# zailaiyiwan123/NOVA_pointcloud

Measured on AMD Instinct MI355X. Metric: generated points/sec/node, NOVA-d48w1024 @2048 pts, 64-step sample, higher is better.
Workload: dtype bf16; 1 GPU; d48w1024_2048pts_b32; ar_steps=64, diffusion_steps=25, batch_per_gpu=32, global_batch=32, guidance=cfg 2-pass, process_group=none

## Files before the change

include/nova_hip.h:

```cpp
#ifndef NOVA_HIP_H_
#define NOVA_HIP_H_

#ifdef __cplusplus
extern "C" {
#endif

#define NOVA_HIP_VERSION 404

typedef enum { NOVA_F32 = 0, NOVA_BF16 = 1, NOVA_F16 = 2 } nova_dtype;
typedef enum { NOVA_ACT_NONE = 0, NOVA_ACT_GELU_ERF = 1, NOVA_ACT_SILU = 2 } nova_act;
typedef enum {
  NOVA_OK = 0,
  NOVA_ERR_ARG = -1,
  NOVA_ERR_SHAPE = -2,
  NOVA_ERR_LAUNCH = -3,
  NOVA_ERR_DEVICE = -4
} nova_status;

int nova_version(void);
const char* nova_last_error(void);
int nova_check_device(void);

#define NOVA_PROF_SLOTS 10
int nova_prof_enable(int on);
int nova_prof_collect(double* ms, double* work, long long* launches, int slots);

int nova_debug_force_gemm_tile(int tile);

int nova_debug_set_attn_variant(int variant);

int nova_debug_set_graphs(int on);
int nova_debug_graph_stats(long* captures, long* replays);
int nova_debug_drop_graphs(void);

int nova_gemm_bias_act(const void* A, const void* W, const float* bias, void* out, int M, int N, int K, int act,
                       int dtype, void* stream);

int nova_quantize_rows_fp8(const void* x_bf16, void* out_fp8, float* scale, long long rows, int D, void* stream);
int nova_gemm_fp8_bias_act(const void* A8, const float* a_scale, const void* W8, const float* w_scale, const float* bias,
                           void* out_bf16, int M, int N, int K, int act, void* stream);

int nova_qkv_rope(const void* x, const void* Wqkv, const float* bias, const float* rope, void* qkv, int S, int L, int D,
                  int heads, int rope_batch, int dtype, void* stream);

int nova_qkv_rope_cols(const void* x, const void* W, const float* bias, const float* rope, void* out, int M, int N, int K,
                       int L, int rope_batch, int head_dim, int rope_cols, int dtype, void* stream);

int nova_rope_table(const float* pos, const long long* ids, float* rope, int nb, int pad, int n_tok, int n_pos, int hd,
                    const float* inv_freq, void* stream);

int nova_attn_fwd(const void* q, const void* k, const void* v, void* o, int S, int heads, int Lq, int Lk, int head_dim,
                  long q_row_stride, long kv_row_stride, long o_row_stride, float scale, int dtype, void* stream);

int nova_attn_fwd_lse(const void* q_scaled, const void* k, const void* v, void* o, float* lse, int S, int heads, int L,
                      int head_dim, long qkv_row_stride, long o_row_stride, const int* key_limit, void* stream);
int nova_attn_bwd(const void* q_scaled, const void* k, const void* v, const void* o, const void* d_o, const float* lse,
                  float* delta_scratch, void* dq, void* dk, void* dv, int S, int heads, int L, int head_dim,
                  long qkv_row_stride, long o_row_stride, long do_row_stride, long dqkv_row_stride, float scale,
                  const int* key_limit, void* stream);

int nova_act_fwd(const void* x, void* y, long long n, int kind, int dtype, void* stream);
int nova_act_bwd(const void* x, const void* dy, void* dx, long long n, int kind, int dtype, void* stream);

int nova_row_norm_bwd(const void* x, const void* dy, const float* gamma, const float* beta, const void* mod, long mod_ld,
                      int scale_off, int shift_off, int gate_off, void* dx, void* dmod, float* dgamma_part, float* dbeta_part,
                      int parts, long rows, int D, float eps, int dtype, void* stream);

int nova_row_norm(const void* in, void* out, const float* gamma, const float* beta, const void* mod, long mod_ld,
                  int scale_off, int shift_off, int gate_off, const void* res, const int* gather, long rows, int D,
                  float eps, int dtype, void* stream);

int nova_row_norm_chain(const void* g, const void* x, const float* gamma, const float* beta, const void* mod, long mod_ld,
                        int gate_off, int scale_off, int shift_off, float eps_first, float eps_second, void* x_new_out,
                        void* h_out, long rows, int D, int dtype, void* stream);

int nova_adaln_fc1(const void* x, const void* mod, long mod_ld, int scale_off, int shift_off, float eps, const void* w,
                   const float* bias, void* h, void* out, long rows, int N, int D, int act, int dtype, void* stream);

int nova_embed_canvas(const float* canvas, const float* mask, const void* w, const float* bias, const void* mask_token,
                      const void* pos_embed, void* z0, int B, int N, int P, int D, int dtype, void* stream);
int nova_build_sequence(const void* prefix, long prefix_seq_rows, const void* tokens, long tok_batch_rows,
                        const long long* ids, void* x, int S, int B, int Lp, int n_sel, int D, int dtype, void* stream);
int nova_scatter_tokens(const void* x1, const long long* ids, void* x2, int S, int B, int Lp, int N, int n_prev, int D,
                        int dtype, void* stream);

int nova_silu_add_rows(const void* a, const void* rowvec, void* out, long rows, int D, int dtype, void* stream);
int nova_timestep_freq(const float* t, const float* freq, void* out, int n, int freq_dim, int dtype, void* stream);
int nova_patch_embed_rows(const float* x, const void* w, const float* bias, void* out, int S, int B, int n, int P, int D,
                          int dtype, void* stream);
int nova_head_cfg_euler(const void* h, const void* w, const float* bias, float* x, int B, int n, int P, int D,
                        float guidance, int cfg, float dt, int dtype, void* stream);

int nova_pointset_nn_dist(const float* x, const float* y, float* d, int B, int N, int M, float clamp_lo, float clamp_hi,
                          int unit_norm, void* stream);
int nova_pointset_pairwise_dist(const float* x, const float* y, float* D, int B, int N, int M, float clamp_lo, float clamp_hi,
                                void* stream);
int nova_pointset_chamfer_matrix(const float* x, const float* y, float* cd, int A, int B, int N, int M, int ldc, int symmetric,
                                 void* stream);
#define NOVA_EMD_MAX_POINTS 4096
int nova_pointset_emd_matrix(const float* x, const float* y, float* emd, int A, int B, int N, int ldc, void* stream);

#define NOVA_OCC_MAX_RES 32
int nova_pointset_occupancy_grid(const float* x, long long* counters, long long* bernoulli, int* node, long long* outside, int S,
                                 int N, int R, int in_sphere, int workgroups, void* stream);

typedef struct {
  const void* qkv_w;
  const float* qkv_b;
  const void* proj_w;
  const float* proj_b;
  const float* norm1_w;
  const float* norm1_b;
  const void* fc1_w;
  const float* fc1_b;
  const void* fc2_w;
  const float* fc2_b;
  const float* norm2_w;
  const float* norm2_b;
} nova_vit_block;

int nova_vit_blocks_forward(const nova_vit_block* blocks, int nblocks, void* x, int S, int L, int D, int heads,
                            int hidden, const float* rope, int rope_batch, void* ws_qkv, void* ws_a, void* ws_b,
                            void* ws_h, int dtype, void* stream);

typedef struct {
  const void* qkv_w8;  const float* qkv_ws;
  const void* fc1_w8;  const float* fc1_ws;
  const void* fc2_w8;  const float* fc2_ws;
} nova_vit_block_fp8;

int nova_row_norm_fp8(const void* in, void* out, const float* gamma, const float* beta, const void* res, void* out8, float* out8_scale,
                      long rows, int D, float eps, void* stream);
int nova_gemm_fp8_gelu_q8(const void* A8, const float* a_scale, const void* W8, const float* w_scale, const float* bias, void* out8,
                          int M, int N, int K, const float* out_scale, unsigned* out_amax, void* stream);
int nova_qkv_rope_fp8(const void* x8, const float* x_scale, const void* w8, const float* w_scale, const float* bias, const float* rope,
                      void* qkv, int S, int L, int D, int heads, int rope_batch, float q_scale, void* stream);

int nova_vit_blocks_forward_fp8(const nova_vit_block* blocks, const nova_vit_block_fp8* q, int nblocks, void* x, int S, int L, int D,
                                int heads, int hidden, const float* rope, int rope_batch, void* ws_qkv, void* ws_a, void* ws_b,
                                void* ws_h, void* ws_x8, float* ws_xs, void* ws_h8, float* ws_hs, float* h_scale, unsigned* h_amax,
                                void* stream);

int nova_vit_blocks_forward_kv(const nova_vit_block* blocks, int nblocks, void* x, int S, int L, int D, int heads,
                               int hidden, const float* rope, int rope_batch, void* kv_cache, long cache_cap,
                               long cache_len, void* ws_qkv, void* ws_a, void* ws_b, void* ws_h, int dtype, void* stream);

int nova_modulate_rows(const void* x, const void* mod, void* out, long rows, int D, int dtype, void* stream);

typedef struct {
  const void* fc1_w;
  const float* fc1_b;
  const void* fc2_w;
  const float* fc2_b;
  const float* norm2_w;
  const float* norm2_b;
} nova_mlp_block;

typedef struct {
  int depth;
  const nova_mlp_block* blocks;
  const void* adaln_w;
  const float* adaln_b;
  const void* patch_w;
  const float* patch_b;
  const void* head_w;
  const float* head_b;
} nova_decoder;

typedef struct {
  float guidance, kx, kv, clip, c0, cx, sigma;
  float extra_scale;
  int extra_kind;
} nova_sampler_step;

int nova_decoder_denoise(const nova_decoder* dec, const void* zc, const void* temb, float* x, const nova_sampler_step* sched,
                         const float* noise, float renorm, float* echo_energy, int steps, int S, int B, int n, int P, int D,
                         void* ws_a, void* ws_u, void* ws_h, void* ws_f, void* ws_g, void* ws_mod, float* ws_v, int mod_steps,
                         int dtype, void* stream);

int nova_decoder_denoise_echo(const nova_decoder* dec, const void* zc, const void* temb, float* x, const nova_sampler_step* sched,
                              const float* noise, float renorm, float* echo_rows, const float* echo_noise, int Ne, int steps, int S, int B,
                              int n, int P, int D, void* ws_a, void* ws_u, void* ws_h, void* ws_f, void* ws_g, void* ws_mod, float* ws_v,
                              int mod_steps, int dtype, void* stream);

#ifdef __cplusplus
}
#endif
#endif
```

nova_pointcloud_amd/csrc/capi.hip:

```cpp
#include <cstdarg>
#include <cstdio>
#include <cstring>
#include <atomic>
#include <cmath>
#include <cstdlib>
#include <mutex>
#include <string>
#include <unordered_map>
#include <utility>
#include <vector>
#include "common.h"
#include "nova_internal.h"

namespace nova {

static thread_local char g_err[512] = "";

int set_error(int code, const char* fmt, ...) {
  va_list ap;
  va_start(ap, fmt);
  vsnprintf(g_err, sizeof(g_err), fmt, ap);
  va_end(ap);
  return code;
}

int check_launch(const char* what) {
  const hipError_t e = hipGetLastError();
  if (e == hipSuccess) return 0;
  return set_error(NOVA_ERR_LAUNCH, "%s: %s", what, hipGetErrorString(e));
}

struct ProfRec { hipEvent_t a, b; int slot; double work; };
static std::atomic<bool> g_prof_on{false};
static std::mutex g_prof_mu;
static std::vector<ProfRec> g_prof;
static std::vector<std::pair<hipEvent_t, hipEvent_t>> g_prof_pool;

ProfScope::ProfScope(int slot, double work, hipStream_t s) : idx(-1), st(s) {
  if (!g_prof_on.load(std::memory_order_relaxed)) return;
  std::lock_guard<std::mutex> lk(g_prof_mu);
  ProfRec r;
  if (!g_prof_pool.empty()) {
    r.a = g_prof_pool.back().first;
    r.b = g_prof_pool.back().second;
    g_prof_pool.pop_back();
  } else if (hipEventCreate(&r.a) != hipSuccess || hipEventCreate(&r.b) != hipSuccess) {
    return;
  }
  r.slot = slot;
  r.work = work;
  (void)hipEventRecord(r.a, st);
  g_prof.push_back(r);
  idx = (int)g_prof.size() - 1;
}
ProfScope::~ProfScope() {
  if (idx < 0) return;
  std::lock_guard<std::mutex> lk(g_prof_mu);
  if (idx < (int)g_prof.size()) (void)hipEventRecord(g_prof[idx].b, st);
}

static inline bool bad_dtype(int dtype) { return dtype != NOVA_F32 && dtype != NOVA_BF16 && dtype != NOVA_F16; }
static inline size_t esize(int dtype) { return dtype_is16(dtype) ? 2 : 4; }

}

using namespace nova;

#define NOVA_REQUIRE(cond, code, ...) \
  do {                                \
    if (!(cond)) return set_error(code, __VA_ARGS__); \
  } while (0)
#define NOVA_TRY(expr)        \
  do {                        \
    const int rc_ = (expr);   \
    if (rc_ != 0) return rc_; \
  } while (0)

namespace nova {
static thread_local bool g_walk_rev = false;
void walk_reverse(bool on) { g_walk_rev = on; }
bool walk_is_reverse() { return g_walk_rev; }
#ifdef NOVA_EXPERIMENTS
static int g_walk_alternate = 1;
void walk_set_alternate(int on) { g_walk_alternate = on; }
#else
constexpr int g_walk_alternate = 1;
#endif
}

extern "C" {

int nova_version(void) { return NOVA_HIP_VERSION; }
const char* nova_last_error(void) { return g_err; }

int nova_check_device(void) {
  int dev = -1;
  if (hipGetDevice(&dev) != hipSuccess) return set_error(NOVA_ERR_DEVICE, "no HIP device");
  hipDeviceProp_t prop;
  if (hipGetDeviceProperties(&prop, dev) != hipSuccess) return set_error(NOVA_ERR_DEVICE, "hipGetDeviceProperties failed");
  if (strncmp(prop.gcnArchName, "gfx950", 6) != 0)
    return set_error(NOVA_ERR_DEVICE, "device %d is %s; libnova_hip is built for gfx950 only", dev, prop.gcnArchName);
  return 0;
}

int nova_debug_force_gemm_tile(int tile) {
  NOVA_REQUIRE(gemm_force_tile(tile) == 0, NOVA_ERR_ARG,
               "force_gemm_tile: this build knows 0 (auto), 16 (small-M kernel; 161 / 162 / 164 with 16 / 32 / 64 rows per workgroup), 64 / 128 (the small-M tile kernels), 256 (persistent), 257 (one tile per workgroup) and 258 (persistent, prologue form); experiment codes need the NOVA_EXPERIMENTS build");
  return 0;
}

int nova_prof_enable(int on) {
  g_prof_on.store(on != 0);
  return 0;
}

int nova_prof_collect(double* ms, double* work, long long* launches, int slots) {
  NOVA_REQUIRE(ms && work && launches && slots >= PROF_SLOTS, NOVA_ERR_ARG, "prof_collect: need %d slots", PROF_SLOTS);
  for (int i = 0; i < slots; ++i) { ms[i] = 0; work[i] = 0; launches[i] = 0; }
  std::lock_guard<std::mutex> lk(g_prof_mu);
  for (auto& r : g_prof) {
    float t = 0.f;
    if (hipEventSynchronize(r.b) == hipSuccess && hipEventElapsedTime(&t, r.a, r.b) == hipSuccess) {
      ms[r.slot] += t;
      work[r.slot] += r.work;
      launches[r.slot] += 1;
    }
    g_prof_pool.emplace_back(r.a, r.b);
  }
  g_prof.clear();
  return 0;
}

int nova_gemm_bias_act(const void* A, const void* W, const float* bias, void* out, int M, int N, int K, int act,
                       int dtype, void* stream) {
  NOVA_REQUIRE(!bad_dtype(dtype), NOVA_ERR_ARG, "gemm: bad dtype %d", dtype);
  NOVA_REQUIRE(M == 0 || (A && W && out), NOVA_ERR_ARG, "gemm: null pointer");
  return gemm_bias_act(A, W, bias, out, M, N, K, act, dtype, (hipStream_t)stream);
}

int nova_quantize_rows_fp8(const void* x, void* out, float* scale, long long rows, int D, void* stream) {
  NOVA_REQUIRE(rows <= 0 || (x && out && scale), NOVA_ERR_ARG, "quantize_rows_fp8: null pointer");
  return quantize_rows_fp8(x, out, scale, (long)rows, D, (hipStream_t)stream);
}

int nova_gemm_fp8_bias_act(const void* A8, const float* a_scale, const void* W8, const float* w_scale, const float* bias,
                           void* out, int M, int N, int K, int act, void* stream) {
  NOVA_REQUIRE(M <= 0 || (A8 && a_scale && W8 && w_scale && out), NOVA_ERR_ARG, "gemm_fp8: null pointer");
  NOVA_REQUIRE(act >= NOVA_ACT_NONE && act <= NOVA_ACT_SILU, NOVA_ERR_ARG, "gemm_fp8: bad activation %d", act);
  return gemm256_fp8_launch(A8, a_scale, W8, w_scale, bias, out, M, N, K, act, (hipStream_t)stream);
}

int nova_qkv_rope(const void* x, const void* Wqkv, const float* bias, const float* rope, void* qkv, int S, int L, int D,
                  int heads, int rope_batch, int dtype, void* stream) {
  NOVA_REQUIRE(!bad_dtype(dtype), NOVA_ERR_ARG, "qkv_rope: bad dtype %d", dtype);
  NOVA_REQUIRE(S * L == 0 || (x && Wqkv && qkv), NOVA_ERR_ARG, "qkv_rope: null pointer");
  return gemm_qkv_rope(x, Wqkv, bias, rope, qkv, S, L, D, heads, rope_batch, dtype, (hipStream_t)stream);
}

int nova_qkv_rope_cols(const void* x, const void* W, const float* bias, const float* rope, void* out, int M, int N, int K,
                       int L, int rope_batch, int head_dim, int rope_cols, int dtype, void* stream) {
  NOVA_REQUIRE(!bad_dtype(dtype), NOVA_ERR_ARG, "qkv_rope_cols: bad dtype %d", dtype);
  NOVA_REQUIRE(M == 0 || (x && W && out), NOVA_ERR_ARG, "qkv_rope_cols: null pointer");
  NOVA_REQUIRE(L > 0 && head_dim > 0 && head_dim % 4 == 0 && rope_cols % 128 == 0 && rope_cols <= N, NOVA_ERR_SHAPE,
               "qkv_rope_cols: bad L/head_dim/rope_cols");
  return gemm_rope_cols(x, W, bias, rope, out, M, N, K, L, rope_batch, head_dim, rope_cols, dtype, (hipStream_t)stream);
}

int nova_rope_table(const float* pos, const long long* ids, float* rope, int nb, int pad, int n_tok, int n_pos, int hd,
                    const float* inv_freq, void* stream) {
  NOVA_REQUIRE(pos && rope && inv_freq, NOVA_ERR_ARG, "rope_table: null pointer");
  NOVA_REQUIRE(hd > 0 && hd % 8 == 0, NOVA_ERR_SHAPE, "rope_table: head_dim %d", hd);
  return rope_table(pos, ids, rope, nb, pad, n_tok, n_pos, hd, inv_freq, (hipStream_t)stream);
}

int nova_attn_fwd(const void* q, const void* k, const void* v, void* o, int S, int heads, int Lq, int Lk, int head_dim,
                  long q_row_stride, long kv_row_stride, long o_row_stride, float scale, int dtype, void* stream) {
  NOVA_REQUIRE(!bad_dtype(dtype), NOVA_ERR_ARG, "attn_fwd: bad dtype %d", dtype);
  NOVA_REQUIRE(q && k && v && o, NOVA_ERR_ARG, "attn_fwd: null pointer");
  return attn_fwd(q, k, v, o, S, heads, Lq, Lk, head_dim, q_row_stride, kv_row_stride, o_row_stride, scale, dtype,
                  (hipStream_t)stream);
}

int nova_attn_fwd_lse(const void* q_scaled, const void* k, const void* v, void* o, float* lse, int S, int heads, int L,
                      int head_dim, long qkv_row_stride, long o_row_stride, const int* key_limit, void* stream) {
  NOVA_REQUIRE(q_scaled && k && v && o && lse, NOVA_ERR_ARG, "attn_fwd_lse: null pointer");
  return attn_fwd(q_scaled, k, v, o, S, heads, L, L, head_dim, qkv_row_stride, qkv_row_stride, o_row_stride, 1.0f, NOVA_BF16,
                  (hipStream_t)stream, true, 0, lse, key_limit);
}

int nova_attn_bwd(const void* q_scaled, const void* k, const void* v, const void* o, const void* d_o, const float* lse,
                  float* delta_scratch, void* dq, void* dk, void* dv, int S, int heads, int L, int head_dim,
                  long qkv_row_stride, long o_row_stride, long do_row_stride, long dqkv_row_stride, float scale,
                  const int* key_limit, void* stream) {
  NOVA_REQUIRE(q_scaled && k && v && o && d_o && lse && delta_scratch && dq && dk && dv, NOVA_ERR_ARG, "attn_bwd: null pointer");
  return attn_bwd(q_scaled, k, v, o, d_o, lse, delta_scratch, dq, dk, dv, S, heads, L, head_dim, qkv_row_stride, o_row_stride,
                  do_row_stride, dqkv_row_stride, scale, (hipStream_t)stream, key_limit);
}

int nova_row_norm(const void* in, void* out, const float* gamma, const float* beta, const void* mod, long mod_ld,
                  int scale_off, int shift_off, int gate_off, const void* res, const int* gather, long rows, int D,
                  float eps, int dtype, void* stream) {
  NOVA_REQUIRE(!bad_dtype(dtype), NOVA_ERR_ARG, "row_norm: bad dtype %d", dtype);
  NOVA_REQUIRE(rows == 0 || (in && out), NOVA_ERR_ARG, "row_norm: null pointer");
  RowNormArgs a{in, out, gamma, beta, mod, mod_ld, scale_off, shift_off, gate_off, res, gather, rows, D, eps};
  return row_norm(a, dtype, (hipStream_t)stream);
}

int nova_row_norm_chain(const void* g, const void* x, const float* gamma, const float* beta, const void* mod, long mod_ld,
                        int gate_off, int scale_off, int shift_off, float eps_first, float eps_second, void* x_new_out,
                        void* h_out, long rows, int D, int dtype, void* stream) {
  NOVA_REQUIRE(dtype_is16(dtype), NOVA_ERR_ARG, "row_norm_chain: dtype %d is not a 16-bit storage type", dtype);
  NOVA_REQUIRE(rows == 0 || (g && x && mod && h_out), NOVA_ERR_ARG, "row_norm_chain: null pointer");
  RowNormArgs a2{g, nullptr, gamma, beta, mod, mod_ld, -1, -1, gate_off, x, nullptr, rows, D, eps_first};
  RowNormArgs a1{nullptr, h_out, nullptr, nullptr, mod, mod_ld, scale_off, shift_off, -1, nullptr, nullptr, rows, D, eps_second};
  return row_norm_chain(a2, a1, x_new_out, dtype, (hipStream_t)stream);
}

int nova_adaln_fc1(const void* x, const void* mod, long mod_ld, int scale_off, int shift_off, float eps, const void* w,
                   const float* bias, void* h, void* out, long rows, int N, int D, int act, int dtype, void* stream) {
  NOVA_REQUIRE(!bad_dtype(dtype), NOVA_ERR_ARG, "adaln_fc1: bad dtype %d", dtype);
  NOVA_REQUIRE(rows == 0 || (x && mod && w && h && out), NOVA_ERR_ARG, "adaln_fc1: null pointer");
  NOVA_REQUIRE(rows >= 0 && rows <= 0x7fffffffL && scale_off >= 0 && shift_off >= 0, NOVA_ERR_ARG, "adaln_fc1: bad rows / offsets");
  RowNormArgs m{x, h, nullptr, nullptr, mod, mod_ld, scale_off, shift_off, -1, nullptr, nullptr, rows, D, eps};
  return gemm_modulate_act(m, w, bias, out, (int)rows, N, D, act, dtype, (hipStream_t)stream);
}

int nova_embed_canvas(const float* canvas, const float* mask, const void* w, const float* bias, const void* mask_token,
                      const void* pos_embed, void* z0, int B, int N, int P, int D, int dtype, void* stream) {
  NOVA_REQUIRE(!bad_dtype(dtype), NOVA_ERR_ARG, "embed_canvas: bad dtype %d", dtype);
  NOVA_REQUIRE(canvas && mask && w && bias && mask_token && z0, NOVA_ERR_ARG, "embed_canvas: null pointer");
  return embed_canvas(canvas, mask, w, bias, mask_token, pos_embed, z0, B, N, P, D, dtype, (hipStream_t)stream);
}

int nova_build_sequence(const void* prefix, long prefix_seq_rows, const void* tokens, long tok_batch_rows,
                        const long long* ids, void* x, int S, int B, int Lp, int n_sel, int D, int dtype, void* stream) {
  NOVA_REQUIRE(!bad_dtype(dtype), NOVA_ERR_ARG, "build_sequence: bad dtype %d", dtype);
  NOVA_REQUIRE(x && (Lp == 0 || prefix) && (n_sel == 0 || tokens) && B > 0, NOVA_ERR_ARG, "build_sequence: null pointer");
  return build_sequence(prefix, prefix_seq_rows, tokens, tok_batch_rows, ids, x, S, B, Lp, n_sel, D, dtype, (hipStream_t)stream);
}

int nova_scatter_tokens(const void* x1, const long long* ids, void* x2, int S, int B, int Lp, int N, int n_prev, int D,
                        int dtype, void* stream) {
  NOVA_REQUIRE(!bad_dtype(dtype), NOVA_ERR_ARG, "scatter_tokens: bad dtype %d", dtype);
  NOVA_REQUIRE(n_prev == 0 || (x1 && ids && x2 && B > 0), NOVA_ERR_ARG, "scatter_tokens: null pointer");
  return scatter_tokens(x1, ids, x2, S, B, Lp, N, n_prev, D, dtype, (hipStream_t)stream);
}

int nova_silu_add_rows(const void* a, const void* rowvec, void* out, long rows, int D, int dtype, void* stream) {
  NOVA_REQUIRE(!bad_dtype(dtype), NOVA_ERR_ARG, "silu_add_rows: bad dtype %d", dtype);
  NOVA_REQUIRE(rows == 0 || (a && out), NOVA_ERR_ARG, "silu_add_rows: null pointer");
  return silu_add_rows(a, rowvec, out, rows, D, dtype, (hipStream_t)stream);
}

int nova_timestep_freq(const float* t, const float* freq, void* out, int n, int freq_dim, int dtype, void* stream) {
  NOVA_REQUIRE(!bad_dtype(dtype), NOVA_ERR_ARG, "timestep_freq: bad dtype %d", dtype);
  NOVA_REQUIRE(t && freq && out && freq_dim % 2 == 0, NOVA_ERR_ARG, "timestep_freq: bad argument");
  return timestep_freq(t, freq, out, n, freq_dim, dtype, (hipStream_t)stream);
}

int nova_patch_embed_rows(const float* x, const void* w, const float* bias, void* out, int S, int B, int n, int P, int D,
                          int dtype, void* stream) {
  NOVA_REQUIRE(!bad_dtype(dtype), NOVA_ERR_ARG, "patch_embed_rows: bad dtype %d", dtype);
  NOVA_REQUIRE(x && w && bias && out && B > 0, NOVA_ERR_ARG, "patch_embed_rows: null pointer");
  return patch_embed_rows(x, w, bias, out, S, B, n, P, D, dtype, (hipStream_t)stream);
}

int nova_head_cfg_euler(const void* h, const void* w, const float* bias, float* x, int B, int n, int P, int D,
                        float guidance, int cfg, float dt, int dtype, void* stream) {
  NOVA_REQUIRE(!bad_dtype(dtype), NOVA_ERR_ARG, "head_cfg_euler: bad dtype %d", dtype);
  NOVA_REQUIRE(h && w && bias && x, NOVA_ERR_ARG, "head_cfg_euler: null pointer");
  NOVA_REQUIRE(!cfg || guidance > 1.0f, NOVA_ERR_ARG, "head_cfg_euler: cfg needs guidance > 1");
  SamplerStep sp{cfg ? guidance : 1.0f, 0.f, 1.f, 0.f, dt, 1.f, 0.f, 0.f, 0};
  return head_cfg_step(h, w, bias, x, nullptr, nullptr, nullptr, nullptr, B, n, P, D, sp, 0, dtype, (hipStream_t)stream);
}


static int vit_blocks(const nova_vit_block* blocks, int nblocks, void* x, int S, int L, int D, int heads, int hidden,
                      const float* rope, int rope_batch, void* ws_qkv, void* ws_a, void* ws_b, void* ws_h, void* cache,
                      long cap, long cache_len, int dtype, hipStream_t st) {
  const int M = S * L, hd = D / heads;
  if (M == 0) return 0;
  const size_t es = esize(dtype);
  const float scale = 1.0f / sqrtf((float)hd);
  const char* qkv = static_cast<const char*>(ws_qkv);
  struct Walk {
    int k = 0;
    void next() { walk_reverse(g_walk_alternate && (k++ & 1)); }
    ~Walk() { walk_reverse(false); }
  } walk;
  for (int i = 0; i < nblocks; ++i) {
    const nova_vit_block& b = blocks[i];
    const bool pre = dtype_is16(dtype);
    walk.next();
    NOVA_TRY(gemm_qkv_rope(x, b.qkv_w, b.qkv_b, rope, ws_qkv, S, L, D, heads, rope_batch, dtype, st,
                           pre ? scale * 1.4426950408889634f : 1.0f));
    walk.next();
    if (cache) {
      char* cb = static_cast<char*>(cache) + (size_t)i * S * cap * 2 * D * es;
      NOVA_TRY(kv_append(ws_qkv, cb, S, L, D, cap, cache_len, dtype, st));
      NOVA_TRY(attn_fwd(qkv, cb, cb + (size_t)D * es, ws_a, S, heads, L, (int)(cache_len + L), hd, 3L * D, 2L * D, D, scale, dtype,
                        st, pre, cap * 2L * D));
    } else {
      NOVA_TRY(attn_fwd(qkv, qkv + (size_t)D * es, qkv + (size_t)2 * D * es, ws_a, S, heads, L, L, hd, 3L * D, 3L * D, D,
                        scale, dtype, st, pre));
    }
    walk.next();
    NOVA_TRY(gemm_bias_act(ws_a, b.proj_w, b.proj_b, ws_b, M, D, D, NOVA_ACT_NONE, dtype, st));
    RowNormArgs n1{ws_b, x, b.norm1_w, b.norm1_b, nullptr, 0, -1, -1, -1, x, nullptr, M, D, 1e-5f};
    walk.next();
    NOVA_TRY(row_norm(n1, dtype, st));
    walk.next();
    NOVA_TRY(gemm_bias_act(x, b.fc1_w, b.fc1_b, ws_h, M, hidden, D, NOVA_ACT_GELU_ERF, dtype, st));
    walk.next();
    NOVA_TRY(gemm_bias_act(ws_h, b.fc2_w, b.fc2_b, ws_b, M, D, hidden, NOVA_ACT_NONE, dtype, st));
    RowNormArgs n2{ws_b, x, b.norm2_w, b.norm2_b, nullptr, 0, -1, -1, -1, x, nullptr, M, D, 1e-5f};
    walk.next();
    NOVA_TRY(row_norm(n2, dtype, st));
  }
  return 0;
}

int nova_vit_blocks_forward(const nova_vit_block* blocks, int nblocks, void* x, int S, int L, int D, int heads,
                            int hidden, const float* rope, int rope_batch, void* ws_qkv, void* ws_a, void* ws_b,
                            void* ws_h, int dtype, void* stream) {
  NOVA_REQUIRE(!bad_dtype(dtype), NOVA_ERR_ARG, "vit_blocks: bad dtype %d", dtype);
  NOVA_REQUIRE(nblocks == 0 || (blocks && x && ws_qkv && ws_a && ws_b && ws_h), NOVA_ERR_ARG, "vit_blocks: null pointer");
  NOVA_REQUIRE(heads > 0 && D % heads == 0, NOVA_ERR_SHAPE, "vit_blocks: D %% heads != 0");
  return vit_blocks(blocks, nblocks, x, S, L, D, heads, hidden, rope, rope_batch, ws_qkv, ws_a, ws_b, ws_h, nullptr, 0, 0, dtype,
                    (hipStream_t)stream);
}

int nova_row_norm_fp8(const void* in, void* out, const float* gamma, const float* beta, const void* res, void* out8, float* out8_scale,
                      long rows, int D, float eps, void* stream) {
  NOVA_REQUIRE(rows == 0 || (in && out && out8 && out8_scale), NOVA_ERR_ARG, "row_norm_fp8: null pointer");
  RowNormArgs a{in, out, gamma, beta, nullptr, 0, -1, -1, -1, res, nullptr, rows, D, eps};
  a.out8 = out8;
  a.out8_scale = out8_scale;
  return row_norm(a, NOVA_BF16, (hipStream_t)stream);
}

int nova_gemm_fp8_gelu_q8(const void* A8, const float* a_scale, const void* W8, const float* w_scale, const float* bias, void* out8,
                          int M, int N, int K, const float* out_scale, unsigned* out_amax, void* stream) {
  NOVA_REQUIRE(M <= 0 || (A8 && a_scale && W8 && w_scale && out8 && out_scale && out_amax), NOVA_ERR_ARG, "gemm_fp8_gelu_q8: null pointer");
  return gemm256_fp8_launch(A8, a_scale, W8, w_scale, bias, out8, M, N, K, NOVA_EPI_GELU_Q8, (hipStream_t)stream, nullptr, 1, 1, 2, 0, 1.0f,
                            0, 0, out_scale, out_amax);
}

int nova_qkv_rope_fp8(const void* x8, const float* x_scale, const void* w8, const float* w_scale, const float* bias, const float* rope,
                      void* qkv, int S, int L, int D, int heads, int rope_batch, float q_scale, void* stream) {
  NOVA_REQUIRE(S * L == 0 || (x8 && x_scale && w8 && w_scale && qkv), NOVA_ERR_ARG, "qkv_rope_fp8: null pointer");
  NOVA_REQUIRE(heads > 0 && D % heads == 0, NOVA_ERR_SHAPE, "qkv_rope_fp8: D %% heads != 0");
  return gemm256_fp8_launch(x8, x_scale, w8, w_scale, bias, qkv, S * L, 3 * D, D, 3, (hipStream_t)stream, rope, L, rope_batch, D / heads,
                            rope ? 2 * D : 0, q_scale, q_scale != 1.0f ? D : 0);
}

int nova_vit_blocks_forward_fp8(const nova_vit_block* blocks, const nova_vit_block_fp8* q, int nblocks, void* x, int S, int L, int D,
                                int heads, int hidden, const float* rope, int rope_batch, void* ws_qkv, void* ws_a, void* ws_b,
                                void* ws_h, void* ws_x8, float* ws_xs, void* ws_h8, float* ws_hs, float* h_scale, unsigned* h_amax,
                                void* stream) {
  NOVA_REQUIRE(nblocks == 0 || (blocks && q && x && ws_qkv && ws_a && ws_b && ws_h && ws_x8 && ws_xs && ws_h8 && ws_hs), NOVA_ERR_ARG,
               "vit_blocks_fp8: null pointer");
  NOVA_REQUIRE((h_scale == nullptr) == (h_amax == nullptr), NOVA_ERR_ARG, "vit_blocks_fp8: h_scale and h_amax come together");
  NOVA_REQUIRE(heads > 0 && D % heads == 0, NOVA_ERR_SHAPE, "vit_blocks_fp8: D %% heads != 0");
  NOVA_REQUIRE(D % 256 == 0 && hidden % 256 == 0, NOVA_ERR_SHAPE, "vit_blocks_fp8: D and hidden must be multiples of 256");
  NOVA_REQUIRE(!rope || L >= 16, NOVA_ERR_SHAPE, "vit_blocks_fp8: L >= 16 with RoPE");
  hipStream_t st = (hipStream_t)stream;
  const int M = S * L, hd = D / heads;
  if (M == 0 || nblocks == 0) return 0;
  const float scale = 1.0f / sqrtf((float)hd);
  const char* qkv = static_cast<const char*>(ws_qkv);
  struct Walk {
    int k = 0;
    void next() { walk_reverse(g_walk_alternate && (k++ & 1)); }
    ~Walk() { walk_reverse(false); }
  } walk;
  NOVA_TRY(quantize_rows_fp8(x, ws_x8, ws_xs, M, D, st));
  for (int i = 0; i < nblocks; ++i) {
    const nova_vit_block& b = blocks[i];
    const nova_vit_block_fp8& w = q[i];
    walk.next();
    NOVA_TRY(gemm256_fp8_launch(ws_x8, ws_xs, w.qkv_w8, w.qkv_ws, b.qkv_b, ws_qkv, M, 3 * D, D, 3 , st, rope, L,
                                rope_batch, hd, rope ? 2 * D : 0, scale * 1.4426950408889634f, D));
    walk.next();
    NOVA_TRY(attn_fwd(qkv, qkv + (size_t)D * 2, qkv + (size_t)2 * D * 2, ws_a, S, heads, L, L, hd, 3L * D, 3L * D, D, scale, NOVA_BF16,
                      st, true));
    walk.next();
    NOVA_TRY(gemm_bias_act(ws_a, b.proj_w, b.proj_b, ws_b, M, D, D, NOVA_ACT_NONE, NOVA_BF16, st));
    RowNormArgs n1{ws_b, x, b.norm1_w, b.norm1_b, nullptr, 0, -1, -1, -1, x, nullptr, M, D, 1e-5f};
    n1.out8 = ws_x8;
    n1.out8_scale = ws_xs;
    walk.next();
    NOVA_TRY(row_norm(n1, NOVA_BF16, st));
    walk.next();
    if (h_scale) {
      NOVA_TRY(gemm256_fp8_launch(ws_x8, ws_xs, w.fc1_w8, w.fc1_ws, b.fc1_b, ws_h8, M, hidden, D, NOVA_EPI_GELU_Q8, st, nullptr, 1, 1, 2, 0,
                                  1.0f, 0, 0, h_scale + i, h_amax + i));
      walk.next();
      NOVA_TRY(gemm256_fp8_launch(ws_h8, h_scale + i, w.fc2_w8, w.fc2_ws, b.fc2_b, ws_b, M, D, hidden, NOVA_ACT_NONE, st, nullptr, 1, 1, 2, 0,
                                  1.0f, 0, 1));
    } else {
      NOVA_TRY(gemm256_fp8_launch(ws_x8, ws_xs, w.fc1_w8, w.fc1_ws, b.fc1_b, ws_h, M, hidden, D, NOVA_ACT_GELU_ERF, st));
      NOVA_TRY(quantize_rows_fp8(ws_h, ws_h8, ws_hs, M, hidden, st));
      walk.next();
      NOVA_TRY(gemm256_fp8_launch(ws_h8, ws_hs, w.fc2_w8, w.fc2_ws, b.fc2_b, ws_b, M, D, hidden, NOVA_ACT_NONE, st));
    }
    RowNormArgs n2{ws_b, x, b.norm2_w, b.norm2_b, nullptr, 0, -1, -1, -1, x, nullptr, M, D, 1e-5f};
    if (i + 1 < nblocks) {
      n2.out8 = ws_x8;
      n2.out8_scale = ws_xs;
    }
    walk.next();
    NOVA_TRY(row_norm(n2, NOVA_BF16, st));
  }
  return 0;
}

int nova_vit_blocks_forward_kv(const nova_vit_block* blocks, int nblocks, void* x, int S, int L, int D, int heads,
                               int hidden, const float* rope, int rope_batch, void* kv_cache, long cache_cap,
                               long cache_len, void* ws_qkv, void* ws_a, void* ws_b, void* ws_h, int dtype, void* stream) {
  NOVA_REQUIRE(!bad_dtype(dtype), NOVA_ERR_ARG, "vit_blocks_kv: bad dtype %d", dtype);
  NOVA_REQUIRE(nblocks == 0 || (blocks && x && kv_cache && ws_qkv && ws_a && ws_b && ws_h), NOVA_ERR_ARG, "vit_blocks_kv: null pointer");
  NOVA_REQUIRE(heads > 0 && D % heads == 0, NOVA_ERR_SHAPE, "vit_blocks_kv: D %% heads != 0");
  NOVA_REQUIRE(cache_len >= 0 && cache_len + L <= cache_cap, NOVA_ERR_SHAPE, "vit_blocks_kv: %ld cached + %d new rows exceed the capacity %ld",
               cache_len, L, cache_cap);
  return vit_blocks(blocks, nblocks, x, S, L, D, heads, hidden, rope, rope_batch, ws_qkv, ws_a, ws_b, ws_h, kv_cache, cache_cap,
                    cache_len, dtype, (hipStream_t)stream);
}

int nova_pointset_nn_dist(const float* x, const float* y, float* d, int B, int N, int M, float clamp_lo, float clamp_hi,
                          int unit_norm, void* stream) {
  NOVA_REQUIRE(B * (long)N == 0 || (x && y && d), NOVA_ERR_ARG, "pointset_nn_dist: null pointer");
  NOVA_REQUIRE(clamp_lo <= clamp_hi, NOVA_ERR_ARG, "pointset_nn_dist: empty clamp range");
  return pointset_nn_dist(x, y, d, B, N, M, clamp_lo, clamp_hi, unit_norm, (hipStream_t)stream);
}

int nova_pointset_pairwise_dist(const float* x, const float* y, float* D, int B, int N, int M, float clamp_lo, float clamp_hi,
                                void* stream) {
  NOVA_REQUIRE(B * (long)N * M == 0 || (x && y && D), NOVA_ERR_ARG, "pointset_pairwise_dist: null pointer");
  NOVA_REQUIRE(clamp_lo <= clamp_hi, NOVA_ERR_ARG, "pointset_pairwise_dist: empty clamp range");
  return pointset_pairwise_dist(x, y, D, B, N, M, clamp_lo, clamp_hi, (hipStream_t)stream);
}

int nova_pointset_chamfer_matrix(const float* x, const float* y, float* cd, int A, int B, int N, int M, int ldc, int symmetric,
                                 void* stream) {
  NOVA_REQUIRE(A <= 0 || B <= 0 || (x && y && cd), NOVA_ERR_ARG, "pointset_chamfer_matrix: null pointer");
  NOVA_REQUIRE(ldc >= B, NOVA_ERR_ARG, "pointset_chamfer_matrix: ldc %d < B %d", ldc, B);
  NOVA_REQUIRE(!symmetric || (x == y && A == B && N == M), NOVA_ERR_ARG,
               "pointset_chamfer_matrix: symmetric mode needs x == y, A == B and N == M");
  return pointset_chamfer_matrix(x, y, cd, A, B, N, M, ldc, symmetric, (hipStream_t)stream);
}

int nova_pointset_emd_matrix(const float* x, const float* y, float* emd, int A, int B, int N, int ldc, void* stream) {
  NOVA_REQUIRE(A <= 0 || B <= 0 || (x && y && emd), NOVA_ERR_ARG, "pointset_emd_matrix: null pointer");
  NOVA_REQUIRE(ldc >= B, NOVA_ERR_ARG, "pointset_emd_matrix: ldc %d < B %d", ldc, B);
  NOVA_REQUIRE(N >= 1 && N <= NOVA_EMD_MAX_POINTS, NOVA_ERR_ARG,
               "pointset_emd_matrix: N %d outside 1 .. %d (the maximum point count NOVA_EMD_MAX_POINTS)", N, NOVA_EMD_MAX_POINTS);
  return pointset_emd_matrix(x, y, emd, A, B, N, ldc, (hipStream_t)stream);
}

int nova_pointset_occupancy_grid(const float* x, long long* counters, long long* bernoulli, int* node, long long* outside, int S,
                                 int N, int R, int in_sphere, int workgroups, void* stream) {
  return pointset_occupancy_grid(x, counters, bernoulli, node, outside, S, N, R, in_sphere, workgroups, (hipStream_t)stream);
}

int nova_modulate_rows(const void* x, const void* mod, void* out, long rows, int D, int dtype, void* stream) {
  NOVA_REQUIRE(!bad_dtype(dtype), NOVA_ERR_ARG, "modulate_rows: bad dtype %d", dtype);
  NOVA_REQUIRE(rows == 0 || (x && mod && out), NOVA_ERR_ARG, "modulate_rows: null pointer");
  return modulate_rows(x, mod, out, rows, D, dtype, (hipStream_t)stream);
}

}

namespace nova {

static int decoder_denoise_launches(const nova_decoder* dec, const void* zc, const void* temb, float* x, const nova_sampler_step* sched,
                                    const float* noise, float renorm, float* echo_energy, int steps, int S, int B, int n, int P, int D,
                                    void* ws_a, void* ws_u, void* ws_h, void* ws_f, void* ws_g, void* ws_mod, float* ws_v, int mod_steps,
                                    int dtype, hipStream_t st, float* echo_rows = nullptr, const float* echo_noise = nullptr, int Ne = 0) {
  const bool do_renorm = renorm < 1.0f;
  const size_t es = esize(dtype);
  const int depth = dec->depth;
  const long mod_ld = (long)(3 * depth + 2) * D;
  const size_t nP = (size_t)B * n * P;
  NOVA_REQUIRE(mod_steps == 1 || mod_steps == steps, NOVA_ERR_ARG, "decoder_denoise: mod_steps must be 1 or steps");
  const bool hoist = mod_steps == steps && steps > 1;
  const long rows_all = (long)S * n;
  if (hoist) {
    NOVA_TRY(silu_add_steps(zc, temb, ws_a, rows_all, steps, D, dtype, st));
    NOVA_TRY(gemm_bias_act(ws_a, dec->adaln_w, dec->adaln_b, ws_mod, (int)(rows_all * steps), (int)mod_ld, D, NOVA_ACT_NONE, dtype, st));
  }
  void* const ws_mod_base = ws_mod;
  for (int i = 0; i < steps; ++i) {
    const SamplerStep sp{sched[i].guidance, sched[i].kx,    sched[i].kv,          sched[i].clip,      sched[i].c0,
                         sched[i].cx,       sched[i].sigma, sched[i].extra_scale, sched[i].extra_kind};
    const int cfg = sp.guidance > 1.0f ? 1 : 0;
    NOVA_REQUIRE(sp.extra_kind >= 0 && sp.extra_kind <= 2, NOVA_ERR_ARG, "decoder_denoise: extra_kind must be 0, 1 or 2");
    const int passes = cfg ? (sp.extra_kind ? 3 : 2) : 1;
    NOVA_REQUIRE(S >= passes * B, NOVA_ERR_SHAPE, "decoder_denoise: step %d needs %d guidance passes but S = %d, B = %d", i, passes, S, B);
    NOVA_REQUIRE(!(do_renorm && cfg) || echo_rows || (sp.kx == 0.f && sp.kv == 1.f && sp.cx == 1.f && sp.sigma == 0.f && sp.clip <= 0.f),
                 NOVA_ERR_ARG, "decoder_denoise: guidance renorm with a scalar echo energy holds for the flow-matching Euler step only "
                 "(other samplers: nova_decoder_denoise_echo with the echo rows)");
    const int Se = passes * B;
    const long rows = (long)Se * n;
    if (hoist) {
      ws_mod = static_cast<char*>(ws_mod_base) + (size_t)i * rows_all * mod_ld * es;
    } else {
      NOVA_TRY(silu_add_rows(zc, static_cast<const char*>(temb) + (size_t)i * D * es, ws_a, rows, D, dtype, st));
      NOVA_TRY(gemm_bias_act(ws_a, dec->adaln_w, dec->adaln_b, ws_mod, (int)rows, (int)mod_ld, D, NOVA_ACT_NONE, dtype, st));
    }
    NOVA_TRY(patch_embed_rows(x, dec->patch_w, dec->patch_b, ws_u, Se, B, n, P, D, dtype, st));
    const bool m1_fused = gemm_modulate_fused((int)rows, D, D, dtype);
    const bool chain = !m1_fused && dtype_is16(dtype);
    for (int b = 0; b < depth; ++b) {
      const nova_mlp_block& blk = dec->blocks[b];
      RowNormArgs m1{ws_u, ws_h, nullptr, nullptr, ws_mod, mod_ld, b * 3 * D, b * 3 * D + D, -1, nullptr, nullptr, rows, D, 1e-6f};
      if (chain && b > 0) {
        NOVA_TRY(gemm_bias_act(ws_h, blk.fc1_w, blk.fc1_b, ws_f, (int)rows, D, D, NOVA_ACT_SILU, dtype, st));
      } else {
        NOVA_TRY(gemm_modulate_act(m1, blk.fc1_w, blk.fc1_b, ws_f, (int)rows, D, D, NOVA_ACT_SILU, dtype, st));
      }
      NOVA_TRY(gemm_bias_act(ws_f, blk.fc2_w, blk.fc2_b, ws_g, (int)rows, D, D, NOVA_ACT_NONE, dtype, st));
      RowNormArgs m2{ws_g, ws_u, blk.norm2_w, blk.norm2_b, ws_mod, mod_ld, -1, -1, b * 3 * D + 2 * D, ws_u, nullptr, rows, D, 1e-5f};
      RowNormArgs mf{ws_u, ws_h, nullptr, nullptr, ws_mod, mod_ld, depth * 3 * D, depth * 3 * D + D, -1, nullptr, nullptr, rows, D, 1e-6f};
      if (b == depth - 1 && dtype_is16(dtype)) {
        NOVA_TRY(row_norm_chain(m2, mf, nullptr, dtype, st));
      } else if (chain) {
        RowNormArgs m1n{ws_u, ws_h, nullptr, nullptr, ws_mod, mod_ld, (b + 1) * 3 * D, (b + 1) * 3 * D + D, -1, nullptr, nullptr, rows, D, 1e-6f};
        NOVA_TRY(row_norm_chain(m2, m1n, ws_u, dtype, st));
      } else {
        NOVA_TRY(row_norm(m2, dtype, st));
        if (b == depth - 1) NOVA_TRY(row_norm(mf, dtype, st));
      }
    }
    const void* head_in = ws_h;
    const float* nz = (noise && sp.sigma != 0.f) ? noise + (size_t)i * nP : nullptr;
    if (do_renorm && echo_rows) {
      const float* enz = (echo_noise && sp.sigma != 0.f) ? echo_noise + (size_t)i * B * Ne * P : nullptr;
      if (cfg) {
        float* extra = passes == 3 ? ws_v + 2 * nP : nullptr;
        NOVA_TRY(head_cfg_step(head_in, dec->head_w, dec->head_b, x, nullptr, ws_v, ws_v + nP, extra, B, n, P, D, sp, 1, dtype, st));
        NOVA_TRY(renorm_step(x, ws_v, ws_v + nP, extra, nz, echo_rows, enz, B, n * P, Ne * P, sp, renorm, 0, st));
      } else {
        NOVA_TRY(head_cfg_step(head_in, dec->head_w, dec->head_b, x, nz, nullptr, nullptr, nullptr, B, n, P, D, sp, 0, dtype, st));
        NOVA_TRY(renorm_step(nullptr, nullptr, nullptr, nullptr, nullptr, echo_rows, enz, B, n * P, Ne * P, sp, renorm, 1, st));
      }
    } else if (do_renorm && cfg) {
      float* extra = passes == 3 ? ws_v + 2 * nP : nullptr;
      NOVA_TRY(head_cfg_step(head_in, dec->head_w, dec->head_b, x, nullptr, ws_v, ws_v + nP, extra, B, n, P, D, sp, 1, dtype, st));
      NOVA_TRY(renorm_euler(x, ws_v, ws_v + nP, extra, echo_energy, B, n, P, sp.c0, renorm, st));
    } else {
      NOVA_TRY(head_cfg_step(head_in, dec->head_w, dec->head_b, x, nz, nullptr, nullptr, nullptr, B, n, P, D, sp, 0, dtype, st));
      if (do_renorm && echo_energy) NOVA_TRY(scale_vector(echo_energy, B, (1.0f + sp.c0) * (1.0f + sp.c0), st));
    }
  }
  return 0;
}


static std::atomic<long> g_graph_epoch{0};
struct DecoderGraphs {
  std::unordered_map<std::string, hipGraphExec_t> execs;
  long captures = 0, replays = 0, epoch = 0;
  ~DecoderGraphs() { clear(false); }
  void clear(bool wait = true) {
    if (wait && !execs.empty()) (void)hipDeviceSynchronize();
    for (auto& kv : execs) (void)hipGraphExecDestroy(kv.second);
    execs.clear();
  }
};
static thread_local DecoderGraphs g_dec_graphs;
static std::atomic<int> g_graphs_on{-1};

static bool graphs_enabled() {
  int v = g_graphs_on.load(std::memory_order_relaxed);
  if (v < 0) {
    const char* e = getenv("NOVA_GRAPHS");
    v = (e && e[0] == '0') ? 0 : 1;
    g_graphs_on.store(v);
  }
  return v != 0;
}

template <typename T> static void key_put(std::string& k, const T& v) { k.append(reinterpret_cast<const char*>(&v), sizeof(T)); }

}

extern "C" {

int nova_debug_set_attn_variant(int variant) {
  NOVA_REQUIRE(attn_set_variant(variant) == 0, NOVA_ERR_ARG, "nova_debug_set_attn_variant: %d is not one of -1 .. 5", variant);
  return 0;
}

int nova_debug_set_graphs(int on) {
  g_graphs_on.store(on ? 1 : 0);
  if (!on) {
    g_graph_epoch.fetch_add(1);
    g_dec_graphs.clear();
  }
  return 0;
}

int nova_debug_drop_graphs(void) {
  g_dec_graphs.clear();
  return 0;
}

int nova_debug_graph_stats(long* captures, long* replays) {
  if (captures) *captures = g_dec_graphs.captures;
  if (replays) *replays = g_dec_graphs.replays;
  return 0;
}

int nova_decoder_denoise(const nova_decoder* dec, const void* zc, const void* temb, float* x, const nova_sampler_step* sched,
                         const float* noise, float renorm, float* echo_energy, int steps, int S, int B, int n, int P, int D,
                         void* ws_a, void* ws_u, void* ws_h, void* ws_f, void* ws_g, void* ws_mod, float* ws_v, int mod_steps,
                         int dtype, void* stream) {
  NOVA_REQUIRE(!bad_dtype(dtype), NOVA_ERR_ARG, "decoder_denoise: bad dtype %d", dtype);
  NOVA_REQUIRE(dec && zc && temb && x && sched && ws_a && ws_u && ws_h && ws_f && ws_g && ws_mod, NOVA_ERR_ARG,
               "decoder_denoise: null pointer");
  NOVA_REQUIRE(S == B || S == 2 * B || S == 3 * B, NOVA_ERR_SHAPE, "decoder_denoise: S must be B, 2B or 3B");
  NOVA_REQUIRE(dec->depth >= 1 && dec->blocks, NOVA_ERR_ARG, "decoder_denoise: the decoder needs at least one block");
  const bool do_renorm = renorm < 1.0f;
  NOVA_REQUIRE(!do_renorm || (echo_energy && ws_v), NOVA_ERR_ARG, "decoder_denoise: renorm needs echo_energy and ws_v");
  if (n == 0 || B == 0) return 0;
  hipStream_t st = (hipStream_t)stream;
  const bool direct = !graphs_enabled() || g_prof_on.load(std::memory_order_relaxed) || noise != nullptr || do_renorm || steps < 2;
  if (direct)
    return decoder_denoise_launches(dec, zc, temb, x, sched, noise, renorm, echo_energy, steps, S, B, n, P, D, ws_a, ws_u, ws_h, ws_f,
                                    ws_g, ws_mod, ws_v, mod_steps, dtype, st);
  if (const long e = g_graph_epoch.load(std::memory_order_relaxed); e != g_dec_graphs.epoch) {
    g_dec_graphs.clear();
    g_dec_graphs.epoch = e;
  }
  std::string key;
  key.reserve(512 + sizeof(nova_sampler_step) * steps + sizeof(nova_mlp_block) * dec->depth);
  key_put(key, *dec);
  for (int b = 0; b < dec->depth; ++b) key_put(key, dec->blocks[b]);
  for (int i = 0; i < steps; ++i) key_put(key, sched[i]);
  const void* ptrs[] = {zc, temb, x, ws_a, ws_u, ws_h, ws_f, ws_g, ws_mod, (const void*)st};
  key_put(key, ptrs);
  const int ints[] = {steps, S, B, n, P, D, mod_steps, dtype, walk_is_reverse() ? 1 : 0, gemm_forced_tile(), skinny_forced_row_blocks()};
  key_put(key, ints);
  auto it = g_dec_graphs.execs.find(key);
  if (it == g_dec_graphs.execs.end()) {
    if (g_dec_graphs.execs.size() >= 2048) g_dec_graphs.clear();
    if (hipStreamBeginCapture(st, hipStreamCaptureModeThreadLocal) != hipSuccess) {
      (void)hipGetLastError();
      return decoder_denoise_launches(dec, zc, temb, x, sched, noise, renorm, echo_energy, steps, S, B, n, P, D, ws_a, ws_u, ws_h, ws_f,
                                      ws_g, ws_mod, ws_v, mod_steps, dtype, st);
    }
    const int rc = decoder_denoise_launches(dec, zc, temb, x, sched, noise, renorm, echo_energy, steps, S, B, n, P, D, ws_a, ws_u, ws_h,
                                            ws_f, ws_g, ws_mod, ws_v, mod_steps, dtype, st);
    hipGraph_t graph = nullptr;
    const hipError_t ec = hipStreamEndCapture(st, &graph);
    if (rc != 0) {
      if (graph) (void)hipGraphDestroy(graph);
      return rc;
    }
    hipGraphExec_t exec = nullptr;
    const hipError_t ei = (ec == hipSuccess && graph) ? hipGraphInstantiate(&exec, graph, nullptr, nullptr, 0) : ec;
    if (graph) (void)hipGraphDestroy(graph);
    if (ei != hipSuccess || !exec) {
      (void)hipGetLastError();
      return decoder_denoise_launches(dec, zc, temb, x, sched, noise, renorm, echo_energy, steps, S, B, n, P, D, ws_a, ws_u, ws_h, ws_f,
                                      ws_g, ws_mod, ws_v, mod_steps, dtype, st);
    }
    it = g_dec_graphs.execs.emplace(std::move(key), exec).first;
    ++g_dec_graphs.captures;
  } else {
    ++g_dec_graphs.replays;
  }
  const hipError_t el = hipGraphLaunch(it->second, st);
  NOVA_REQUIRE(el == hipSuccess, NOVA_ERR_LAUNCH, "decoder_denoise: hipGraphLaunch failed: %s", hipGetErrorString(el));
  return 0;
}

int nova_decoder_denoise_echo(const nova_decoder* dec, const void* zc, const void* temb, float* x, const nova_sampler_step* sched,
                              const float* noise, float renorm, float* echo_rows, const float* echo_noise, int Ne, int steps, int S, int B,
                              int n, int P, int D, void* ws_a, void* ws_u, void* ws_h, void* ws_f, void* ws_g, void* ws_mod, float* ws_v,
                              int mod_steps, int dtype, void* stream) {
  NOVA_REQUIRE(!bad_dtype(dtype), NOVA_ERR_ARG, "decoder_denoise_echo: bad dtype %d", dtype);
  NOVA_REQUIRE(dec && zc && temb && x && sched && ws_a && ws_u && ws_h && ws_f && ws_g && ws_mod, NOVA_ERR_ARG,
               "decoder_denoise_echo: null pointer");
  NOVA_REQUIRE(S == B || S == 2 * B || S == 3 * B, NOVA_ERR_SHAPE, "decoder_denoise_echo: S must be B, 2B or 3B");
  NOVA_REQUIRE(dec->depth >= 1 && dec->blocks, NOVA_ERR_ARG, "decoder_denoise_echo: the decoder needs at least one block");
  NOVA_REQUIRE(renorm < 1.0f && echo_rows && ws_v && Ne >= 0, NOVA_ERR_ARG,
               "decoder_denoise_echo: for guidance_renorm < 1 with the echo rows given (else: nova_decoder_denoise)");
  if (n == 0 || B == 0) return 0;
  return decoder_denoise_launches(dec, zc, temb, x, sched, noise, renorm, nullptr, steps, S, B, n, P, D, ws_a, ws_u, ws_h, ws_f, ws_g, ws_mod,
                                  ws_v, mod_steps, dtype, (hipStream_t)stream, echo_rows, echo_noise, Ne);
}

}
```

nova_pointcloud_amd/csrc/gemm.hip:

```cpp
#include <cstdlib>
#include "common.h"
#include "nova_internal.h"

namespace nova {

constexpr int ROWB = 128;

struct GemmEpi {
  const float* bias;
  const float* rope;
  int L;
  int rope_batch;
  int hd;
  int rope_cols;
  float q_scale;
  int q_cols;
};

enum { EPI_NONE = 0, EPI_GELU = 1, EPI_SILU = 2, EPI_ROPE = 3 };

template <typename T> struct Frag;
template <> struct Frag<bf16_t> { u4v v; };
template <> struct Frag<f16_t> { u4v v; };
template <> struct Frag<float> { f4v v; };

__device__ __forceinline__ f4v mma(const Frag<bf16_t>& w, const Frag<bf16_t>& a, f4v c) { return Half16<bf16_t>::mfma16(w.v, a.v, c); }
__device__ __forceinline__ f4v mma(const Frag<f16_t>& w, const Frag<f16_t>& a, f4v c) { return Half16<f16_t>::mfma16(w.v, a.v, c); }
__device__ __forceinline__ f4v mma(const Frag<float>& w, const Frag<float>& a, f4v c) {
#pragma unroll
  for (int j = 0; j < 4; ++j) c = __builtin_amdgcn_mfma_f32_16x16x4f32(w.v[j], a.v[j], c, 0, 0, 0);
  return c;
}

template <typename T>
__device__ __forceinline__ Frag<T> lds_frag(const char* tile, int row, int chunk) {
  const int phys = chunk ^ ((row >> 1) & 7);
  Frag<T> f;
  f.v = *reinterpret_cast<const decltype(f.v)*>(tile + row * ROWB + phys * 16);
  return f;
}

#ifndef NOVA_GEMM64_STAGES
#define NOVA_GEMM64_STAGES 2
#endif
template <typename T, int EPI, int F = 4>
__global__ __launch_bounds__(256, 2) void gemm_kernel(const T* __restrict__ A, const T* __restrict__ W,
                                                       T* __restrict__ C, int M, int N, int K, int ntm,
                                                       int ntn, GemmEpi e) {
  constexpr int BM = 32 * F, BN = 32 * F, TILE_BYTES = BM * ROWB, WT = 16 * F;
  constexpr int NST = F == 2 ? NOVA_GEMM64_STAGES : 2;
  __shared__ __attribute__((aligned(16))) char smem[NST * 2 * TILE_BYTES];
  const int tid = threadIdx.x, lane = tid & 63, wid = tid >> 6;
  const int wm = wid >> 1, wn = wid & 1;

  const int nwg = ntm * ntn;
  const int t = xcd_remap(blockIdx.x, nwg);
  constexpr int GM = 8;
  const int per_group = GM * ntn;
  const int group = t / per_group, first_m = group * GM;
  const int gsz = min(ntm - first_m, GM);
  const int tm = first_m + (t % per_group) % gsz;
  const int tn = (t % per_group) / gsz;
  const int m0 = tm * BM, n0 = tn * BN;

  const int rr = lane >> 3, cp = lane & 7;
  const char* a_src[4];
  const char* w_src[4];
  const size_t rowbytes = (size_t)K * sizeof(T);
#pragma unroll
  for (int i = 0; i < F; ++i) {
    const int row = (wid * F + i) * 8 + rr;
    const int c = cp ^ ((row >> 1) & 7);
    const int am = min(m0 + row, M - 1);
    a_src[i] = reinterpret_cast<const char*>(A) + (size_t)am * rowbytes + c * 16;
    w_src[i] = reinterpret_cast<const char*>(W) + (size_t)(n0 + row) * rowbytes + c * 16;
  }
  auto stage = [&](int buf, int kt) {
    char* la = smem + buf * 2 * TILE_BYTES + wid * F * 1024;
    char* lw = la + TILE_BYTES;
#pragma unroll
    for (int i = 0; i < F; ++i) {
      __builtin_amdgcn_global_load_lds(a_src[i] + (size_t)kt * ROWB, NOVA_LDS_PTR(la + i * 1024), 16, 0, 0);
      __builtin_amdgcn_global_load_lds(w_src[i] + (size_t)kt * ROWB, NOVA_LDS_PTR(lw + i * 1024), 16, 0, 0);
    }
  };

  const int nkt = K / (ROWB / (int)sizeof(T));
  const int fr = lane & 15, fg = lane >> 4;

  f4v bv[F];
#pragma unroll
  for (int nf = 0; nf < F; ++nf) bv[nf] = f4v{0.f, 0.f, 0.f, 0.f};
  if (e.bias) {
#pragma unroll
    for (int nf = 0; nf < F; ++nf) bv[nf] = *reinterpret_cast<const f4v*>(e.bias + n0 + wn * WT + nf * 16 + fg * 4);
  }
  f4v acc[F][F];
#pragma unroll
  for (int i = 0; i < F; ++i)
#pragma unroll
    for (int j = 0; j < F; ++j) acc[i][j] = bv[i];

#pragma unroll
  for (int s = 0; s < NST - 1; ++s)
    if (s < nkt) stage(s, s);
  for (int kt = 0; kt < nkt; ++kt) {
    if constexpr (NST == 2) {
      asm volatile("s_waitcnt vmcnt(0)" ::: "memory");
    } else {
      const int young = min(NST - 2, nkt - 1 - kt);
      if (young >= 3) asm volatile("s_waitcnt vmcnt(%0)" ::"n"(3 * 2 * F) : "memory");
      else if (young == 2) asm volatile("s_waitcnt vmcnt(%0)" ::"n"(2 * 2 * F) : "memory");
      else if (young == 1) asm volatile("s_waitcnt vmcnt(%0)" ::"n"(1 * 2 * F) : "memory");
      else asm volatile("s_waitcnt vmcnt(0)" ::: "memory");
    }
    if constexpr (NST == 2) __syncthreads();
    else asm volatile("s_barrier" ::: "memory");
    if (kt + NST - 1 < nkt) stage((kt + NST - 1) % NST, kt + NST - 1);
    const char* ta = smem + (kt % NST) * 2 * TILE_BYTES;
    const char* tw = ta + TILE_BYTES;
#pragma unroll
    for (int kk = 0; kk < 2; ++kk) {
      Frag<T> af[F], wf[F];
#pragma unroll
      for (int f = 0; f < F; ++f) {
        af[f] = lds_frag<T>(ta, wm * WT + f * 16 + fr, fg + 4 * kk);
        wf[f] = lds_frag<T>(tw, wn * WT + f * 16 + fr, fg + 4 * kk);
      }
#pragma unroll
      for (int nf = 0; nf < F; ++nf)
#pragma unroll
        for (int mf = 0; mf < F; ++mf) acc[nf][mf] = mma(wf[nf], af[mf], acc[nf][mf]);
    }
  }

  const bool rot = EPI == EPI_ROPE && n0 < e.rope_cols;
#pragma unroll
  for (int mf = 0; mf < F; ++mf) {
    const int m = m0 + wm * WT + mf * 16 + fr;
    if (m >= M) continue;
    f4v cs[F];
    if (rot) {
      const int s = m / e.L, l = m - s * e.L;
      const float* ropem = e.rope + ((size_t)(s % e.rope_batch) * e.L + l) * e.hd;
#pragma unroll
      for (int nf = 0; nf < F; ++nf) cs[nf] = *reinterpret_cast<const f4v*>(ropem + (n0 + wn * WT + nf * 16 + fg * 4) % e.hd);
    }
    T* dst = C + (size_t)m * N + n0 + wn * WT + fg * 4;
#pragma unroll
    for (int nf = 0; nf < F; ++nf) {
      f4v v = acc[nf][mf];
      if (EPI == EPI_GELU) {
#pragma unroll
        for (int j = 0; j < 4; ++j) v[j] = sizeof(T) == 2 ? v[j] : gelu_erf(v[j]);
        if (sizeof(T) == 2) v = gelu_erf_fast4(v);
      } else if (EPI == EPI_SILU) {
#pragma unroll
        for (int j = 0; j < 4; ++j) v[j] = silu(v[j]);
      } else if (EPI == EPI_ROPE) {
        if (rot) {
          v = rope_rotate4(v, cs[nf]);
        }
        if (n0 < e.q_cols) v = v * e.q_scale;
      }
      if constexpr (sizeof(T) == 2) {
        u2v o = {Half16<T>::pack(v[0], v[1]), Half16<T>::pack(v[2], v[3])};
        *reinterpret_cast<u2v*>(dst + nf * 16) = o;
      } else {
        *reinterpret_cast<f4v*>(dst + nf * 16) = v;
      }
    }
  }
}

int gemm256_launch(const void* A, const void* W, void* C, int M, int N, int K, int epi, const float* bias,
                   const float* rope, int L, int rope_batch, int hd, int rope_cols, float q_scale, int q_cols, int dtype,
                   hipStream_t st, int form = 0);
int gemm256_cu_count();

static thread_local int g_force_tile = 0;
#ifdef NOVA_EXPERIMENTS
void gemm256_set_variant(int v);
void gemm256_set_gm(int g);
void gemm256_set_stagger(int cycles);
void gemm256_set_grid(int n);
void walk_set_alternate(int on);
#endif
int gemm_forced_tile() { return g_force_tile; }
int gemm_force_tile(int tile) {
#ifdef NOVA_EXPERIMENTS
  if (tile == 50000 || tile == 50001) {
    walk_set_alternate(tile - 50000);
    return 0;
  }
  if (tile >= 40000 && tile <= 40512) {
    gemm256_set_grid(tile - 40000);
    return 0;
  }
  if (tile >= 30000 && tile < 31000) {
    gemm256_set_stagger((tile - 30000) * 256);
    return 0;
  }
  if (tile >= 7001 && tile <= 7064) {
    gemm256_set_gm(tile - 7000);
    return 0;
  }
  if (tile >= 2560 && tile <= 2580) {
    gemm256_set_variant(tile - 2560);
    tile = 256;
  }
#endif
  if (tile == 161 || tile == 162 || tile == 164) {
    skinny_force_row_blocks(tile - 160);
    tile = 16;
  } else {
    skinny_force_row_blocks(0);
  }
  if (tile != 0 && tile != 16 && tile != 64 && tile != 128 && tile != 256 && tile != 257 && tile != 258) return -1;
  g_force_tile = tile;
  return 0;
}

static long min_tiles256() {
  static const long v = [] {
    const char* e = getenv("NOVA_GEMM_MIN_TILES");
    return e && *e ? atol(e) : (long)gemm256_cu_count() / 2;
  }();
  return v;
}

template <typename T>
static int launch_gemm(const void* A, const void* W, void* C, int M, int N, int K, int epi, const GemmEpi& e,
                       hipStream_t st) {
  const int kelems = ROWB / (int)sizeof(T);
  if (M <= 0) return 0;
  if (N % 128 != 0 || K % kelems != 0 || K <= 0)
    return set_error(NOVA_ERR_SHAPE, "gemm: need N %% 128 == 0 and K %% %d == 0 (got M=%d N=%d K=%d)", kelems, M, N, K);
  const bool can256 = N % 256 == 0 && (epi != EPI_ROPE || (e.rope_cols % 256 == 0 && e.q_cols % 256 == 0));
  if (g_force_tile >= 256 && !can256) return set_error(NOVA_ERR_SHAPE, "gemm: 256-tile kernel needs N %% 256 == 0");
  const long tiles256 = (long)((M + 255) / 256) * (N / 256);
  if (can256 && (g_force_tile >= 256 || (g_force_tile == 0 && M >= 4096 && tiles256 >= min_tiles256())))
    return gemm256_launch(A, W, C, M, N, K, epi, e.bias, e.rope, e.L, e.rope_batch, e.hd, e.rope_cols, e.q_scale, e.q_cols,
                          dtype_of<T>(), st, g_force_tile == 257 ? 1 : g_force_tile == 258 ? 2 : 0);
  constexpr int BM = 128, BN = 128;
  int ntm = (M + BM - 1) / BM, ntn = N / BN;
  ProfScope prof(PROF_GEMM_SMALL, 2.0 * M * N * K, st);
  const T* a = static_cast<const T*>(A);
  const T* w = static_cast<const T*>(W);
  T* c = static_cast<T*>(C);
  static const bool tile64_ok = [] { const char* v = getenv("NOVA_GEMM_TILE64"); return !(v && v[0] == '0'); }();
  if (g_force_tile == 64 || (tile64_ok && g_force_tile == 0 && epi != EPI_ROPE && (long)ntm * ntn * 4 <= (long)gemm256_cu_count() * 3)) {
    if (epi == EPI_ROPE) return set_error(NOVA_ERR_SHAPE, "gemm: the 64 tile has no RoPE epilogue");
    ntm = (M + 63) / 64;
    ntn = N / 64;
    dim3 grid64(ntm * ntn), block(256);
    switch (epi) {
      case EPI_NONE: hipLaunchKernelGGL((gemm_kernel<T, EPI_NONE, 2>), grid64, block, 0, st, a, w, c, M, N, K, ntm, ntn, e); break;
      case EPI_GELU: hipLaunchKernelGGL((gemm_kernel<T, EPI_GELU, 2>), grid64, block, 0, st, a, w, c, M, N, K, ntm, ntn, e); break;
      case EPI_SILU: hipLaunchKernelGGL((gemm_kernel<T, EPI_SILU, 2>), grid64, block, 0, st, a, w, c, M, N, K, ntm, ntn, e); break;
      default: return set_error(NOVA_ERR_ARG, "gemm: unknown epilogue %d", epi);
    }
    return check_launch("gemm (64 tile)");
  }
  dim3 grid(ntm * ntn), block(256);
  switch (epi) {
    case EPI_NONE: hipLaunchKernelGGL((gemm_kernel<T, EPI_NONE>), grid, block, 0, st, a, w, c, M, N, K, ntm, ntn, e); break;
    case EPI_GELU: hipLaunchKernelGGL((gemm_kernel<T, EPI_GELU>), grid, block, 0, st, a, w, c, M, N, K, ntm, ntn, e); break;
    case EPI_SILU: hipLaunchKernelGGL((gemm_kernel<T, EPI_SILU>), grid, block, 0, st, a, w, c, M, N, K, ntm, ntn, e); break;
    case EPI_ROPE: hipLaunchKernelGGL((gemm_kernel<T, EPI_ROPE>), grid, block, 0, st, a, w, c, M, N, K, ntm, ntn, e); break;
    default: return set_error(NOVA_ERR_ARG, "gemm: unknown epilogue %d", epi);
  }
  return check_launch("gemm");
}

int gemm_bias_act(const void* A, const void* W, const float* bias, void* out, int M, int N, int K, int act,
                  int dtype, hipStream_t st) {
  GemmEpi e{bias, nullptr, 1, 1, 2, 0, 1.0f, 0};
  if (act < 0 || act > 2) return set_error(NOVA_ERR_ARG, "gemm: unknown activation %d", act);
  if (dtype_is16(dtype) && (g_force_tile == 16 || (g_force_tile == 0 && skinny_gemm_fits(M, N, K, false))))
    return skinny_gemm(A, W, bias, out, M, N, K, act, nullptr, dtype, st);
  return dispatch_dtype(dtype, [&](auto tag) { return launch_gemm<decltype(tag)>(A, W, out, M, N, K, act, e, st); });
}

bool gemm_modulate_fused(int M, int N, int K, int dtype) {
  return dtype_is16(dtype) && (g_force_tile == 16 || (g_force_tile == 0 && skinny_gemm_fits(M, N, K, true)));
}

int gemm_modulate_act(const RowNormArgs& pro, const void* W, const float* bias, void* out, int M, int N, int K, int act,
                      int dtype, hipStream_t st) {
  if (gemm_modulate_fused(M, N, K, dtype)) return skinny_gemm(nullptr, W, bias, out, M, N, K, act, &pro, dtype, st);
  if (int rc = row_norm(pro, dtype, st)) return rc;
  return gemm_bias_act(pro.out, W, bias, out, M, N, K, act, dtype, st);
}

int gemm_qkv_rope(const void* x, const void* Wqkv, const float* bias, const float* rope, void* qkv, int S, int L,
                  int D, int heads, int rope_batch, int dtype, hipStream_t st, float q_scale) {
  const int hd = D / heads;
  if (heads <= 0 || D % heads != 0 || hd % 4 != 0) return set_error(NOVA_ERR_SHAPE, "qkv_rope: bad heads/D");
  const int epi = (rope || q_scale != 1.0f) ? EPI_ROPE : EPI_NONE;
  if (rope && rope_batch <= 0) return set_error(NOVA_ERR_ARG, "qkv_rope: rope_batch must be > 0");
  GemmEpi e{bias, rope, L, rope ? rope_batch : 1, hd, rope ? 2 * D : 0, q_scale, q_scale != 1.0f ? D : 0};
  return dispatch_dtype(dtype, [&](auto tag) { return launch_gemm<decltype(tag)>(x, Wqkv, qkv, S * L, 3 * D, D, epi, e, st); });
}

int gemm_rope_cols(const void* x, const void* W, const float* bias, const float* rope, void* out, int M, int N, int K,
                   int L, int rope_batch, int hd, int rope_cols, int dtype, hipStream_t st) {
  if (rope && rope_batch <= 0) return set_error(NOVA_ERR_ARG, "rope_cols: rope_batch must be > 0");
  GemmEpi e{bias, rope, L, rope ? rope_batch : 1, hd, rope_cols, 1.0f, 0};
  const int epi = rope ? EPI_ROPE : EPI_NONE;
  return dispatch_dtype(dtype, [&](auto tag) { return launch_gemm<decltype(tag)>(x, W, out, M, N, K, epi, e, st); });
}

}
```

nova_pointcloud_amd/csrc/nova_internal.h:

```cpp
#pragma once
#include <hip/hip_runtime.h>
#include "../../include/nova_hip.h"

#include "common.h"

namespace nova {

template <typename T> constexpr int dtype_of() { return sizeof(T) == 4 ? NOVA_F32 : NOVA_BF16; }
template <> constexpr int dtype_of<f16_t>() { return NOVA_F16; }
inline bool dtype_is16(int dtype) { return dtype == NOVA_BF16 || dtype == NOVA_F16; }
template <typename F> inline auto dispatch_dtype(int dtype, F&& f) {
  return dtype == NOVA_BF16 ? f(bf16_t{}) : dtype == NOVA_F16 ? f(f16_t{}) : f(float{});
}
template <typename F> inline auto dispatch_half(int dtype, F&& f) { return dtype == NOVA_F16 ? f(f16_t{}) : f(bf16_t{}); }

int set_error(int code, const char* fmt, ...) __attribute__((format(printf, 2, 3)));
int check_launch(const char* what);

enum { PROF_GEMM_NONE = 0, PROF_GEMM_GELU, PROF_GEMM_SILU, PROF_GEMM_ROPE, PROF_ATTN, PROF_ROWNORM, PROF_GEMM_SMALL, PROF_GEMM_WIDEK,
       PROF_TOKENS, PROF_DECODER, PROF_SLOTS };
inline int prof_gemm_slot(int epi, int N, int K) { return epi == 0 && K > N ? PROF_GEMM_WIDEK : PROF_GEMM_NONE + epi; }
struct ProfScope {
  ProfScope(int slot, double work, hipStream_t st);
  ~ProfScope();
  int idx;
  hipStream_t st;
};

int gemm_bias_act(const void* A, const void* W, const float* bias, void* out, int M, int N, int K, int act,
                  int dtype, hipStream_t st);
int gemm_qkv_rope(const void* x, const void* Wqkv, const float* bias, const float* rope, void* qkv, int S, int L,
                  int D, int heads, int rope_batch, int dtype, hipStream_t st, float q_scale = 1.0f);

int gemm_rope_cols(const void* x, const void* W, const float* bias, const float* rope, void* out, int M, int N, int K,
                   int L, int rope_batch, int hd, int rope_cols, int dtype, hipStream_t st);
int gemm_force_tile(int tile);
int gemm_forced_tile();
void walk_reverse(bool on);
bool walk_is_reverse();

int attn_fwd(const void* q, const void* k, const void* v, void* o, int S, int heads, int Lq, int Lk, int hd,
             long q_row_stride, long kv_row_stride, long o_row_stride, float scale, int dtype, hipStream_t st,
             bool q_prescaled = false, long kv_seq_stride = 0, float* lse = nullptr, const int* klim = nullptr);
int attn_fwd_m16(const void* q, const void* k, const void* v, void* o, int S, int heads, int Lq, int Lk, int hd, long q_rs, long kv_rs,
                 long o_rs, float cl, int dtype, hipStream_t st, long kv_ss, float* lse, int rows_per_wave, bool sum_on_mfma, bool pipelined = false,
                 const int* klim = nullptr);
constexpr int NOVA_ATTN_DEFAULT_VARIANT = 3;
int attn_set_variant(int v);
int attn_variant();
int attn_bwd(const void* q, const void* k, const void* v, const void* o, const void* d_o, const float* lse, float* delta, void* dq,
             void* dk, void* dv, int S, int heads, int L, int hd, long qkv_rs, long o_rs, long do_rs, long dqkv_rs, float scale,
             hipStream_t st, const int* klim = nullptr);

struct RowNormArgs {
  const void* in;
  void* out;
  const float* gamma;
  const float* beta;
  const void* mod;
  long mod_ld;
  int scale_off, shift_off, gate_off;
  const void* res;
  const int* gather;
  long rows;
  int D;
  float eps;
  int rev = 0;
  void* out8 = nullptr;
  float* out8_scale = nullptr;
};
int row_norm(const RowNormArgs& a, int dtype, hipStream_t st);

bool skinny_gemm_fits(int M, int N, int K, bool modulate);
bool gemm_modulate_fused(int M, int N, int K, int dtype);
int skinny_forced_row_blocks();
void skinny_force_row_blocks(int rb);
int skinny_gemm(const void* A, const void* W, const float* bias, void* out, int M, int N, int K, int act,
                const RowNormArgs* pro, int dtype, hipStream_t st);
int row_norm_chain(const RowNormArgs& a2, const RowNormArgs& a1, void* x_new_out, int dtype, hipStream_t st);
int gemm_modulate_act(const RowNormArgs& pro, const void* W, const float* bias, void* out, int M, int N, int K, int act,
                      int dtype, hipStream_t st);

int rope_table(const float* pos, const long long* ids, float* table, int nb, int pad, int n_tok, int n_pos,
               int hd, const float* inv_freq, hipStream_t st);
int embed_canvas(const float* canvas, const float* mask, const void* w, const float* bias, const void* mask_token,
                 const void* pos_embed, void* z0, int B, int N, int P, int D, int dtype, hipStream_t st);
int build_sequence(const void* prefix, long prefix_seq_rows, const void* tokens, long tok_batch_rows,
                   const long long* ids, void* x, int S, int B, int Lp, int n_sel, int D, int dtype, hipStream_t st);
int scatter_tokens(const void* x1, const long long* ids, void* x2, int S, int B, int Lp, int N, int n_prev, int D,
                   int dtype, hipStream_t st);
int quantize_rows_fp8(const void* x, void* out, float* scale, long rows, int D, hipStream_t st);
int gemm256_fp8_launch(const void* A8, const float* sa, const void* W8, const float* sw, const float* bias, void* C, int M,
                       int N, int K, int epi, hipStream_t st, const float* rope = nullptr, int L = 1, int rope_batch = 1,
                       int hd = 2, int rope_cols = 0, float q_scale = 1.0f, int q_cols = 0, int sa_scalar = 0,
                       const float* q8_scale = nullptr, unsigned* q8_amax = nullptr);
constexpr int NOVA_EPI_GELU_Q8 = 5;
int silu_add_rows(const void* a, const void* rowvec, void* out, long rows, int D, int dtype, hipStream_t st);
int silu_add_steps(const void* a, const void* vecs, void* out, long rows, int nvec, int D, int dtype, hipStream_t st);
int timestep_freq(const float* t, const float* freq, void* out, int n, int freq_dim, int dtype, hipStream_t st);
int patch_embed_rows(const float* x, const void* w, const float* bias, void* out, int S, int B, int n, int P, int D,
                     int dtype, hipStream_t st);
struct SamplerStep {
  float guidance, kx, kv, clip, c0, cx, sigma;
  float extra_scale;
  int extra_kind;
};
int head_cfg_step(const void* h, const void* w, const float* bias, float* x, const float* noise, float* vhat, float* cond,
                  float* extra, int B, int n, int P, int D, const SamplerStep& sp, int defer, int dtype, hipStream_t st);
int scale_vector(float* v, int n, float f, hipStream_t st);
int renorm_euler(float* x, const float* vhat, const float* cond, const float* extra, float* echo, int B, int n, int P, float dt,
                 float renorm, hipStream_t st);
int renorm_step(float* x, const float* vhat, const float* cond, const float* extra, const float* noise, float* echo, const float* echo_noise,
                int B, int nP, int eP, const SamplerStep& sp, float renorm, int echo_only, hipStream_t st);
int kv_append(const void* qkv, void* cache, int S, int Lq, int D, long cap, long base, int dtype, hipStream_t st);
int modulate_rows(const void* x, const void* mod, void* out, long rows, int D, int dtype, hipStream_t st);


int pointset_nn_dist(const float* x, const float* y, float* d, int B, int N, int M, float lo, float hi, int unit, hipStream_t st);
int pointset_pairwise_dist(const float* x, const float* y, float* D, int B, int N, int M, float lo, float hi, hipStream_t st);
int pointset_chamfer_matrix(const float* x, const float* y, float* cd, int A, int B, int N, int M, int ldc, int symmetric,
                            hipStream_t st);
int pointset_emd_matrix(const float* x, const float* y, float* emd, int A, int B, int N, int ldc, hipStream_t st);
int pointset_occupancy_grid(const float* x, long long* counters, long long* bernoulli, int* node, long long* outside, int S, int N,
                            int R, int in_sphere, int workgroups, hipStream_t st);

}
```

nova_pointcloud_amd/csrc/rowops.hip:

```cpp
#include "common.h"
#include "nova_internal.h"
#include "rownorm.h"

namespace nova {

template <typename T> struct Vec4;
template <> struct Vec4<float> {
  static __device__ __forceinline__ f4v load(const float* p) { return *reinterpret_cast<const f4v*>(p); }
  static __device__ __forceinline__ void store(float* p, f4v v) { *reinterpret_cast<f4v*>(p) = v; }
};
template <typename T> struct Vec4Half {
  static __device__ __forceinline__ f4v load(const T* p) {
    const u2v u = *reinterpret_cast<const u2v*>(p);
    const f2v a = Half16<T>::unpack(u[0]), b = Half16<T>::unpack(u[1]);
    return f4v{a[0], a[1], b[0], b[1]};
  }
  static __device__ __forceinline__ void store(T* p, f4v v) {
    u2v u = {Half16<T>::pack(v[0], v[1]), Half16<T>::pack(v[2], v[3])};
    *reinterpret_cast<u2v*>(p) = u;
  }
};
template <> struct Vec4<bf16_t> : Vec4Half<bf16_t> {};
template <> struct Vec4<f16_t> : Vec4Half<f16_t> {};

template <typename T, int NIT, bool HAS_RES, bool HAS_MOD>
__global__ __launch_bounds__(256) void row_norm_kernel(RowNormArgs a) {
  using C = Chunk<T>;
  constexpr int NV = C::N / 4;
  const int lane = threadIdx.x & 63;
  const long row = (long)xcd_remap_dir(blockIdx.x, gridDim.x, a.rev != 0) * 4 + (threadIdx.x >> 6);
  if (row >= a.rows) return;
  C x[NIT];
  row_norm_compute<T, NIT, HAS_RES, HAS_MOD>(a, row, lane, x);
  T* out = static_cast<T*>(a.out) + row * a.D;
  const bool q8 = sizeof(T) == 2 && a.out8 != nullptr;
  float amax = 0.f;
#pragma unroll
  for (int it = 0; it < NIT; ++it) {
    const int d = (it * 64 + lane) * C::N;
    if (d < a.D) {
      x[it].store(out + d);
      if (q8) {
        x[it] = x[it].rounded();
#pragma unroll
        for (int k = 0; k < NV; ++k)
#pragma unroll
          for (int j = 0; j < 4; ++j) amax = fmaxf(amax, fabsf(x[it].v[k][j]));
      }
    }
  }
  if constexpr (sizeof(T) == 2) {
    if (q8) {
      amax = wave_max(amax);
      const float sc = amax > 0.f ? amax * (1.0f / 448.0f) : 1.0f;
      const float inv = 1.0f / sc;
      if (lane == 0) a.out8_scale[row] = sc;
      uint8_t* o8 = static_cast<uint8_t*>(a.out8) + row * a.D;
#pragma unroll
      for (int it = 0; it < NIT; ++it) {
        const int d = (it * 64 + lane) * C::N;
        if (d < a.D) {
          u2v o;
#pragma unroll
          for (int k = 0; k < 2; ++k) {
            int w = 0;
            w = __builtin_amdgcn_cvt_pk_fp8_f32(x[it].v[k % NV][0] * inv, x[it].v[k % NV][1] * inv, w, false);
            w = __builtin_amdgcn_cvt_pk_fp8_f32(x[it].v[k % NV][2] * inv, x[it].v[k % NV][3] * inv, w, true);
            o[k] = (uint32_t)w;
          }
          *reinterpret_cast<u2v*>(o8 + d) = o;
        }
      }
    }
  }
}

template <typename T, int NIT>
static void launch_row_norm(const RowNormArgs& a, dim3 grid, hipStream_t st) {
  const bool r = a.res != nullptr, m = a.mod != nullptr;
  if (r && m) hipLaunchKernelGGL((row_norm_kernel<T, NIT, true, true>), grid, dim3(256), 0, st, a);
  else if (r) hipLaunchKernelGGL((row_norm_kernel<T, NIT, true, false>), grid, dim3(256), 0, st, a);
  else if (m) hipLaunchKernelGGL((row_norm_kernel<T, NIT, false, true>), grid, dim3(256), 0, st, a);
  else hipLaunchKernelGGL((row_norm_kernel<T, NIT, false, false>), grid, dim3(256), 0, st, a);
}

int row_norm(const RowNormArgs& a, int dtype, hipStream_t st) {
  if (a.rows <= 0) return 0;
  const int vec = dtype_is16(dtype) ? 8 : 4;
  if (a.D % vec != 0 || a.D > 2048) return set_error(NOVA_ERR_SHAPE, "row_norm: D=%d unsupported (need D %% %d == 0, D <= 2048)", a.D, vec);
  if (a.mod && (a.mod_ld % vec || (a.scale_off >= 0 && (a.scale_off % vec || a.shift_off % vec || a.shift_off < 0)) ||
                (a.gate_off >= 0 && a.gate_off % vec)))
    return set_error(NOVA_ERR_SHAPE, "row_norm: modulation offsets must be multiples of %d", vec);
  if ((a.gamma == nullptr) != (a.beta == nullptr)) return set_error(NOVA_ERR_ARG, "row_norm: gamma/beta must come together");
  if (a.out8 && (dtype != NOVA_BF16 || !a.out8_scale)) return set_error(NOVA_ERR_ARG, "row_norm: the fp8 side output needs bf16 rows and a scale buffer");
  dim3 grid((unsigned)((a.rows + 3) / 4));
  RowNormArgs ar = a;
  ar.rev = walk_is_reverse() ? 1 : 0;
  const double esz = dtype_is16(dtype) ? 2.0 : 4.0;
  const int nmod = a.mod ? ((a.scale_off >= 0 ? 2 : 0) + (a.gate_off >= 0 ? 1 : 0)) : 0;
  ProfScope prof(PROF_ROWNORM, esz * a.rows * a.D * (2.0 + (a.res ? 1 : 0) + nmod), st);
  const int chunks = (a.D / vec + 63) / 64;
  if (dtype_is16(dtype)) {
    dispatch_half(dtype, [&](auto tag) {
      if (chunks <= 2) launch_row_norm<decltype(tag), 2>(ar, grid, st);
      else launch_row_norm<decltype(tag), 4>(ar, grid, st);
      return 0;
    });
  } else {
    if (chunks <= 4) launch_row_norm<float, 4>(ar, grid, st);
    else launch_row_norm<float, 8>(ar, grid, st);
  }
  return check_launch("row_norm");
}

template <typename T, int NIT>
__global__ __launch_bounds__(256) void row_norm_chain_kernel(RowNormArgs a2, RowNormArgs a1, T* __restrict__ x_new_out) {
  const int lane = threadIdx.x & 63;
  const long row = (long)blockIdx.x * 4 + (threadIdx.x >> 6);
  if (row >= a2.rows) return;
  RowChainRegs<T, NIT> g;
  row_chain_load<T, NIT>(a2, a1, row, lane, g);
  u4v xn[NIT];
  Chunk<T> y[NIT];
  row_chain_finish<T, NIT>(a2, a1, lane, g, xn, y);
  T* out = static_cast<T*>(a1.out) + row * a1.D;
#pragma unroll
  for (int it = 0; it < NIT; ++it) {
    const int d = (it * 64 + lane) * 8;
    if (d < a1.D) {
      y[it].store(out + d);
      if (x_new_out) *reinterpret_cast<u4v*>(x_new_out + row * a1.D + d) = xn[it];
    }
  }
}

int row_norm_chain(const RowNormArgs& a2, const RowNormArgs& a1, void* x_new_out, int dtype, hipStream_t st) {
  if (a2.rows <= 0) return 0;
  if (!dtype_is16(dtype)) return set_error(NOVA_ERR_ARG, "row_norm_chain: 16-bit rows only");
  if (a2.D != a1.D || a2.rows != a1.rows || a2.D % 8 || a2.D > 2048) return set_error(NOVA_ERR_SHAPE, "row_norm_chain: bad shapes");
  if (!a2.in || !a2.res || !a2.mod || a2.gate_off < 0 || a2.scale_off >= 0 || a2.gather || !a1.mod || a1.scale_off < 0 || a1.shift_off < 0 ||
      a1.gate_off >= 0 || a1.gamma || a1.res || a1.gather || !a1.out || (a2.gamma == nullptr) != (a2.beta == nullptr))
    return set_error(NOVA_ERR_ARG, "row_norm_chain: first norm = gate + residual, second = scale / shift modulate");
  if (a2.mod_ld % 8 || a2.gate_off % 8 || a1.mod_ld % 8 || a1.scale_off % 8 || a1.shift_off % 8)
    return set_error(NOVA_ERR_SHAPE, "row_norm_chain: modulation offsets must be multiples of 8");
  const dim3 grid((unsigned)((a2.rows + 3) / 4));
  ProfScope prof(PROF_ROWNORM, 2.0 * a2.rows * a2.D * 6.0, st);
  dispatch_half(dtype, [&](auto tag) {
    using T = decltype(tag);
    if ((a2.D / 8 + 63) / 64 <= 2) hipLaunchKernelGGL((row_norm_chain_kernel<T, 2>), grid, dim3(256), 0, st, a2, a1, static_cast<T*>(x_new_out));
    else hipLaunchKernelGGL((row_norm_chain_kernel<T, 4>), grid, dim3(256), 0, st, a2, a1, static_cast<T*>(x_new_out));
    return 0;
  });
  return check_launch("row_norm_chain");
}

__global__ void rope_table_kernel(const float* __restrict__ pos, const long long* __restrict__ ids,
                                  float* __restrict__ table, int nb, int pad, int n_tok, int n_pos, int hd,
                                  const float* __restrict__ inv_freq) {
  const int half = hd / 2;
  const long total = (long)nb * (pad + n_tok) * half;
  const int n0 = (hd / 8) / 2, n1 = ((hd - hd / 8) / 2) / 2;
  for (long i = (long)blockIdx.x * blockDim.x + threadIdx.x; i < total; i += (long)gridDim.x * blockDim.x) {
    const int p = (int)(i % half);
    const long bl = i / half;
    const int l = (int)(bl % (pad + n_tok)), b = (int)(bl / (pad + n_tok));
    float cs = 1.f, sn = 0.f;
    if (l >= pad) {
      const int tok = l - pad;
      long idx = ids ? ids[(long)b * n_tok + tok] : tok;
      idx = idx < 0 ? 0 : (idx >= n_pos ? n_pos - 1 : idx);
      const int axis = p < n0 ? 0 : (p < n0 + n1 ? 1 : 2);
      const float ang = pos[idx * 3 + axis] * inv_freq[p];
      cs = cosf(ang);
      sn = sinf(ang);
    }
    table[2 * i] = cs;
    table[2 * i + 1] = sn;
  }
}

int rope_table(const float* pos, const long long* ids, float* table, int nb, int pad, int n_tok, int n_pos, int hd,
               const float* inv_freq, hipStream_t st) {
  ProfScope prof(PROF_TOKENS, 0.0, st);
  const long total = (long)nb * (pad + n_tok) * (hd / 2);
  if (total <= 0) return 0;
  const int blocks = (int)((total + 255) / 256 > 4096 ? 4096 : (total + 255) / 256);
  hipLaunchKernelGGL(rope_table_kernel, dim3(blocks), dim3(256), 0, st, pos, ids, table, nb, pad, n_tok, n_pos, hd, inv_freq);
  return check_launch("rope_table");
}

template <typename T>
__global__ __launch_bounds__(256) void embed_canvas_kernel(const float* __restrict__ canvas, const float* __restrict__ mask,
                                                           const T* __restrict__ w, const float* __restrict__ bias,
                                                           const T* __restrict__ mask_token, const T* __restrict__ pos_embed,
                                                           T* __restrict__ z0, int N, int P, int D) {
  __shared__ float xs[64];
  const long tok = blockIdx.x;
  if (threadIdx.x < P) xs[threadIdx.x] = canvas[tok * P + threadIdx.x];
  __syncthreads();
  const float m = mask[tok];
  const int n = (int)(tok % N);
  for (int d = threadIdx.x; d < D; d += 256) {
    float e = bias[d];
    for (int p = 0; p < P; ++p) e += xs[p] * to_f<T>(w[(long)d * P + p]);
    float z = e * (1.0f - m) + to_f<T>(mask_token[d]) * m;
    if (pos_embed) z += to_f<T>(pos_embed[(long)n * D + d]);
    z0[tok * D + d] = from_f<T>(z);
  }
}

int embed_canvas(const float* canvas, const float* mask, const void* w, const float* bias, const void* mask_token,
                 const void* pos_embed, void* z0, int B, int N, int P, int D, int dtype, hipStream_t st) {
  ProfScope prof(PROF_TOKENS, 0.0, st);
  if ((long)B * N <= 0) return 0;
  if (P > 64 || P <= 0) return set_error(NOVA_ERR_SHAPE, "embed_canvas: patch vector length %d unsupported (1..64)", P);
  dim3 grid((unsigned)((long)B * N)), block(256);
  dispatch_dtype(dtype, [&](auto tag) {
    using T = decltype(tag);
    hipLaunchKernelGGL(embed_canvas_kernel<T>, grid, block, 0, st, canvas, mask, (const T*)w, bias, (const T*)mask_token, (const T*)pos_embed, (T*)z0, N, P, D);
    return 0;
  });
  return check_launch("embed_canvas");
}

template <typename T>
__global__ __launch_bounds__(256) void build_sequence_kernel(const T* __restrict__ prefix, long prefix_seq_rows,
                                                             const T* __restrict__ tokens, long tok_batch_rows,
                                                             const long long* __restrict__ ids, T* __restrict__ x,
                                                             long rows, int B, int Lp, int n_sel, int D) {
  const int lane = threadIdx.x & 63;
  const long row = (long)blockIdx.x * 4 + (threadIdx.x >> 6);
  if (row >= rows) return;
  const int L = Lp + n_sel;
  const long s = row / L;
  const int l = (int)(row - s * L);
  const T* src;
  if (l < Lp) {
    src = prefix + (s * prefix_seq_rows + l) * D;
  } else {
    const int b = (int)(s % B);
    const long j = ids ? (long)ids[(long)b * n_sel + (l - Lp)] : (long)(l - Lp);
    src = tokens + ((long)b * tok_batch_rows + j) * D;
  }
  T* dst = x + row * D;
  constexpr int V = 16 / sizeof(T);
  for (int d = lane * V; d < D; d += 64 * V) *reinterpret_cast<u4v*>(dst + d) = *reinterpret_cast<const u4v*>(src + d);
}

int build_sequence(const void* prefix, long prefix_seq_rows, const void* tokens, long tok_batch_rows,
                   const long long* ids, void* x, int S, int B, int Lp, int n_sel, int D, int dtype, hipStream_t st) {
  ProfScope prof(PROF_TOKENS, 0.0, st);
  const long rows = (long)S * (Lp + n_sel);
  if (rows <= 0) return 0;
  const int V = dtype_is16(dtype) ? 8 : 4;
  if (D % V) return set_error(NOVA_ERR_SHAPE, "build_sequence: D must be a multiple of %d", V);
  dim3 grid((unsigned)((rows + 3) / 4)), block(256);
  dispatch_dtype(dtype, [&](auto tag) {
    using T = decltype(tag);
    hipLaunchKernelGGL(build_sequence_kernel<T>, grid, block, 0, st, (const T*)prefix, prefix_seq_rows, (const T*)tokens, tok_batch_rows, ids, (T*)x, rows, B, Lp, n_sel, D);
    return 0;
  });
  return check_launch("build_sequence");
}

template <typename T>
__global__ __launch_bounds__(256) void scatter_tokens_kernel(const T* __restrict__ x1, const long long* __restrict__ ids,
                                                             T* __restrict__ x2, long rows, int B, int Lp, int N,
                                                             int n_prev, int D) {
  const int lane = threadIdx.x & 63;
  const long row = (long)blockIdx.x * 4 + (threadIdx.x >> 6);
  if (row >= rows) return;
  const long s = row / n_prev;
  const int j = (int)(row - s * n_prev);
  const int b = (int)(s % B);
  const long tgt = (long)ids[(long)b * n_prev + j];
  const T* src = x1 + (s * (Lp + n_prev) + Lp + j) * D;
  T* dst = x2 + (s * (Lp + N) + Lp + tgt) * D;
  constexpr int V = 16 / sizeof(T);
  for (int d = lane * V; d < D; d += 64 * V) *reinterpret_cast<u4v*>(dst + d) = *reinterpret_cast<const u4v*>(src + d);
}

int scatter_tokens(const void* x1, const long long* ids, void* x2, int S, int B, int Lp, int N, int n_prev, int D,
                   int dtype, hipStream_t st) {
  ProfScope prof(PROF_TOKENS, 0.0, st);
  const long rows = (long)S * n_prev;
  if (rows <= 0) return 0;
  const int V = dtype_is16(dtype) ? 8 : 4;
  if (D % V) return set_error(NOVA_ERR_SHAPE, "scatter_tokens: D must be a multiple of %d", V);
  dim3 grid((unsigned)((rows + 3) / 4)), block(256);
  dispatch_dtype(dtype, [&](auto tag) {
    using T = decltype(tag);
    hipLaunchKernelGGL(scatter_tokens_kernel<T>, grid, block, 0, st, (const T*)x1, ids, (T*)x2, rows, B, Lp, N, n_prev, D);
    return 0;
  });
  return check_launch("scatter_tokens");
}

template <typename T>
__global__ __launch_bounds__(256) void silu_add_rows_kernel(const T* __restrict__ a, const T* __restrict__ vec,
                                                            T* __restrict__ out, long total4, int D) {
  for (long i = (long)blockIdx.x * blockDim.x + threadIdx.x; i < total4; i += (long)gridDim.x * blockDim.x) {
    const long e = i * 4;
    const int d = (int)(e % D);
    f4v x = Vec4<T>::load(a + e);
    if (vec) x = x + Vec4<T>::load(vec + d);
#pragma unroll
    for (int j = 0; j < 4; ++j) x[j] = silu(x[j]);
    Vec4<T>::store(out + e, x);
  }
}

__global__ __launch_bounds__(256) void quantize_rows_fp8_kernel(const bf16_t* __restrict__ x, uint8_t* __restrict__ out,
                                                                float* __restrict__ scale, long rows, int D) {
  using C = Chunk<bf16_t>;
  constexpr int NIT = 16;
  const int lane = threadIdx.x & 63;
  const long row = (long)blockIdx.x * 4 + (threadIdx.x >> 6);
  if (row >= rows) return;
  const bf16_t* in = x + row * D;
  C v[NIT];
  float amax = 0.f;
#pragma unroll
  for (int it = 0; it < NIT; ++it) {
    const int d = (it * 64 + lane) * 8;
    if (d < D) {
      v[it] = C::load(in + d);
#pragma unroll
      for (int k = 0; k < 2; ++k)
#pragma unroll
        for (int j = 0; j < 4; ++j) amax = fmaxf(amax, fabsf(v[it].v[k][j]));
    }
  }
  amax = wave_max(amax);
  const float sc = amax > 0.f ? amax * (1.0f / 448.0f) : 1.0f;
  const float inv = 1.0f / sc;
  if (lane == 0) scale[row] = sc;
#pragma unroll
  for (int it = 0; it < NIT; ++it) {
    const int d = (it * 64 + lane) * 8;
    if (d < D) {
      u2v o;
#pragma unroll
      for (int k = 0; k < 2; ++k) {
        int w = 0;
        w = __builtin_amdgcn_cvt_pk_fp8_f32(v[it].v[k][0] * inv, v[it].v[k][1] * inv, w, false);
        w = __builtin_amdgcn_cvt_pk_fp8_f32(v[it].v[k][2] * inv, v[it].v[k][3] * inv, w, true);
        o[k] = (uint32_t)w;
      }
      *reinterpret_cast<u2v*>(out + row * D + d) = o;
    }
  }
}

int quantize_rows_fp8(const void* x, void* out, float* scale, long rows, int D, hipStream_t st) {
  ProfScope prof(PROF_TOKENS, 0.0, st);
  if (rows <= 0) return 0;
  if (D % 8 != 0 || D > 8192) return set_error(NOVA_ERR_SHAPE, "quantize_rows_fp8: need D %% 8 == 0 and D <= 8192 (got %d)", D);
  hipLaunchKernelGGL(quantize_rows_fp8_kernel, dim3((unsigned)((rows + 3) / 4)), dim3(256), 0, st, (const bf16_t*)x, (uint8_t*)out, scale,
                     rows, D);
  return check_launch("quantize_rows_fp8");
}

template <typename T>
__global__ __launch_bounds__(256) void silu_add_steps_kernel(const T* __restrict__ a, const T* __restrict__ vecs, T* __restrict__ out,
                                                             long per_step4, long total4, int D) {
  for (long i = (long)blockIdx.x * blockDim.x + threadIdx.x; i < total4; i += (long)gridDim.x * blockDim.x) {
    const long step = i / per_step4, e = (i - step * per_step4) * 4;
    const int d = (int)(e % D);
    f4v x = Vec4<T>::load(a + e) + Vec4<T>::load(vecs + step * D + d);
#pragma unroll
    for (int j = 0; j < 4; ++j) x[j] = silu(x[j]);
    Vec4<T>::store(out + i * 4, x);
  }
}

int silu_add_steps(const void* a, const void* vecs, void* out, long rows, int nvec, int D, int dtype, hipStream_t st) {
  ProfScope prof(PROF_DECODER, 0.0, st);
  if (rows <= 0 || nvec <= 0) return 0;
  if (D % 4) return set_error(NOVA_ERR_SHAPE, "silu_add_steps: D %% 4 != 0");
  const long per4 = rows * D / 4, total4 = per4 * nvec;
  const int blocks = (int)((total4 + 255) / 256 > 16384 ? 16384 : (total4 + 255) / 256);
  dispatch_dtype(dtype, [&](auto tag) {
    using T = decltype(tag);
    hipLaunchKernelGGL(silu_add_steps_kernel<T>, dim3(blocks), dim3(256), 0, st, (const T*)a, (const T*)vecs, (T*)out, per4, total4, D);
    return 0;
  });
  return check_launch("silu_add_steps");
}

int silu_add_rows(const void* a, const void* rowvec, void* out, long rows, int D, int dtype, hipStream_t st) {
  ProfScope prof(PROF_DECODER, 0.0, st);
  if (rows <= 0) return 0;
  if (D % 4) return set_error(NOVA_ERR_SHAPE, "silu_add_rows: D %% 4 != 0");
  const long total4 = rows * D / 4;
  const int blocks = (int)((total4 + 255) / 256 > 8192 ? 8192 : (total4 + 255) / 256);
  dispatch_dtype(dtype, [&](auto tag) {
    using T = decltype(tag);
    hipLaunchKernelGGL(silu_add_rows_kernel<T>, dim3(blocks), dim3(256), 0, st, (const T*)a, (const T*)rowvec, (T*)out, total4, D);
    return 0;
  });
  return check_launch("silu_add_rows");
}

template <typename T>
__global__ void timestep_freq_kernel(const float* __restrict__ t, const float* __restrict__ freq, T* __restrict__ out,
                                     int n, int F) {
  const int half = F / 2;
  for (int i = blockIdx.x * blockDim.x + threadIdx.x; i < n * half; i += gridDim.x * blockDim.x) {
    const int row = i / half, kf = i % half;
    const float ang = t[row] * freq[kf];
    out[(long)row * F + kf] = from_f<T>(cosf(ang));
    out[(long)row * F + half + kf] = from_f<T>(sinf(ang));
  }
}

int timestep_freq(const float* t, const float* freq, void* out, int n, int freq_dim, int dtype, hipStream_t st) {
  ProfScope prof(PROF_DECODER, 0.0, st);
  if (n <= 0) return 0;
  const int total = n * (freq_dim / 2);
  dispatch_dtype(dtype, [&](auto tag) {
    using T = decltype(tag);
    hipLaunchKernelGGL(timestep_freq_kernel<T>, dim3((total + 255) / 256), dim3(256), 0, st, t, freq, (T*)out, n, freq_dim);
    return 0;
  });
  return check_launch("timestep_freq");
}

template <typename T>
__global__ __launch_bounds__(256) void patch_embed_rows_kernel(const float* __restrict__ x, const T* __restrict__ w,
                                                               const float* __restrict__ bias, T* __restrict__ out,
                                                               int B, int n, int P, int D) {
  __shared__ float xs[64];
  const long row = blockIdx.x;
  const long s = row / n;
  const int j = (int)(row - s * n), b = (int)(s % B);
  if (threadIdx.x < P) xs[threadIdx.x] = x[((long)b * n + j) * P + threadIdx.x];
  __syncthreads();
  for (int d = threadIdx.x; d < D; d += 256) {
    float e = bias[d];
    for (int p = 0; p < P; ++p) e += xs[p] * to_f<T>(w[(long)d * P + p]);
    out[row * D + d] = from_f<T>(e);
  }
}

int patch_embed_rows(const float* x, const void* w, const float* bias, void* out, int S, int B, int n, int P, int D,
                     int dtype, hipStream_t st) {
  ProfScope prof(PROF_DECODER, 0.0, st);
  if ((long)S * n <= 0) return 0;
  if (P > 64 || P <= 0) return set_error(NOVA_ERR_SHAPE, "patch_embed_rows: patch vector length %d unsupported", P);
  dim3 grid((unsigned)((long)S * n)), block(256);
  dispatch_dtype(dtype, [&](auto tag) {
    using T = decltype(tag);
    hipLaunchKernelGGL(patch_embed_rows_kernel<T>, grid, block, 0, st, x, (const T*)w, bias, (T*)out, B, n, P, D);
    return 0;
  });
  return check_launch("patch_embed_rows");
}

template <typename T>
__global__ __launch_bounds__(256) void head_cfg_step_kernel(const T* __restrict__ h, const T* __restrict__ w,
                                                            const float* __restrict__ bias, float* __restrict__ x,
                                                            const float* __restrict__ noise, float* __restrict__ vhat,
                                                            float* __restrict__ cond, float* __restrict__ extra, long rows, int B,
                                                            int n, int P, int D, SamplerStep sp, int defer) {
  const int lane = threadIdx.x & 63;
  const long row = (long)blockIdx.x * 4 + (threadIdx.x >> 6);
  if (row >= rows) return;
  const int cfg = sp.guidance > 1.0f;
  const int kind = cfg ? sp.extra_kind : 0;
  const T* hc = h + row * D;
  const T* hu = h + ((long)B * n + row) * D;
  const T* h3 = h + ((long)2 * B * n + row) * D;
  for (int p = 0; p < P; ++p) {
    float ac = 0.f, au = 0.f, a3 = 0.f;
    for (int d = lane * 4; d < D; d += 256) {
      const f4v wv = Vec4<T>::load(w + (long)p * D + d);
      const f4v c4 = Vec4<T>::load(hc + d);
      ac += (wv[0] * c4[0] + wv[1] * c4[1]) + (wv[2] * c4[2] + wv[3] * c4[3]);
      if (cfg) {
        const f4v u4 = Vec4<T>::load(hu + d);
        au += (wv[0] * u4[0] + wv[1] * u4[1]) + (wv[2] * u4[2] + wv[3] * u4[3]);
      }
      if (kind) {
        const f4v t4 = Vec4<T>::load(h3 + d);
        a3 += (wv[0] * t4[0] + wv[1] * t4[1]) + (wv[2] * t4[2] + wv[3] * t4[3]);
      }
    }
    ac = wave_sum(ac) + bias[p];
    float vv = ac, ex = 0.f;
    if (cfg) {
      au = wave_sum(au) + bias[p];
      if (kind) a3 = wave_sum(a3) + bias[p];
      if (kind == 1) {
        vv = au + (ac - a3) * sp.guidance;
        ex = (a3 - au) * sp.extra_scale;
      } else {
        vv = au + (ac - au) * sp.guidance;
        if (kind == 2) ex = (ac - a3) * sp.extra_scale;
      }
    }
    if (lane == 0) {
      const long e = row * P + p;
      if (defer) {
        vhat[e] = vv;
        cond[e] = ac;
        if (extra) extra[e] = ex;
      } else {
        vv += ex;
        const float xo = x[e];
        float x0 = sp.kx * xo + sp.kv * vv;
        if (sp.clip > 0.f) x0 = fminf(fmaxf(x0, -sp.clip), sp.clip);
        float xn = sp.c0 * x0 + sp.cx * xo;
        if (noise) xn += sp.sigma * noise[e];
        x[e] = xn;
      }
    }
  }
}

int head_cfg_step(const void* h, const void* w, const float* bias, float* x, const float* noise, float* vhat, float* cond,
                  float* extra, int B, int n, int P, int D, const SamplerStep& sp, int defer, int dtype, hipStream_t st) {
  ProfScope prof(PROF_DECODER, 0.0, st);
  const long rows = (long)B * n;
  if (rows <= 0) return 0;
  if (D % 4) return set_error(NOVA_ERR_SHAPE, "head_cfg_step: D %% 4 != 0");
  if (defer && (!vhat || !cond)) return set_error(NOVA_ERR_ARG, "head_cfg_step: deferred mode needs vhat and cond buffers");
  if (sp.extra_kind < 0 || sp.extra_kind > 2) return set_error(NOVA_ERR_ARG, "head_cfg_step: extra_kind must be 0, 1 or 2");
  if (defer && sp.extra_kind && sp.guidance > 1.0f && !extra) return set_error(NOVA_ERR_ARG, "head_cfg_step: deferred 3-pass mode needs the extra buffer");
  dim3 grid((unsigned)((rows + 3) / 4)), block(256);
  dispatch_dtype(dtype, [&](auto tag) {
    using T = decltype(tag);
    hipLaunchKernelGGL(head_cfg_step_kernel<T>, grid, block, 0, st, (const T*)h, (const T*)w, bias, x, noise, vhat, cond, extra, rows, B, n, P, D, sp, defer);
    return 0;
  });
  return check_launch("head_cfg_step");
}

__global__ __launch_bounds__(256) void renorm_euler_kernel(float* __restrict__ x, const float* __restrict__ vhat,
                                                          const float* __restrict__ cond, const float* __restrict__ extra,
                                                          float* __restrict__ echo, int nP, float dt, float renorm) {
  __shared__ float red[2][4];
  const int b = blockIdx.x, lane = threadIdx.x & 63, wv = threadIdx.x >> 6;
  const float* vb = vhat + (long)b * nP;
  const float* cb = cond + (long)b * nP;
  float sv = 0.f, sc = 0.f;
  for (int i = threadIdx.x; i < nP; i += 256) {
    sv += vb[i] * vb[i];
    sc += cb[i] * cb[i];
  }
  sv = wave_sum(sv);
  sc = wave_sum(sc);
  if (lane == 0) { red[0][wv] = sv; red[1][wv] = sc; }
  __syncthreads();
  const float E = echo[b];
  const float nx = sqrtf((red[0][0] + red[0][1]) + (red[0][2] + red[0][3]) + E);
  const float nc = sqrtf((red[1][0] + red[1][1]) + (red[1][2] + red[1][3]) + E);
  const float ratio = fminf(fmaxf(nc / nx, renorm), 1.0f);
  for (int i = threadIdx.x; i < nP; i += 256) x[(long)b * nP + i] += dt * (ratio * vb[i] + (extra ? extra[(long)b * nP + i] : 0.f));
  __syncthreads();
  if (threadIdx.x == 0) {
    const float f = 1.0f + dt * ratio;
    echo[b] = E * f * f;
  }
}

__global__ __launch_bounds__(256) void renorm_step_kernel(float* __restrict__ x, const float* __restrict__ vhat, const float* __restrict__ cond,
                                                         const float* __restrict__ extra, const float* __restrict__ noise,
                                                         float* __restrict__ echo, const float* __restrict__ echo_noise, int nP, int eP,
                                                         SamplerStep sp, float renorm, int echo_only) {
  __shared__ float red[3][4];
  const int b = blockIdx.x, lane = threadIdx.x & 63, wv = threadIdx.x >> 6;
  float* eb = echo + (long)b * eP;
  float ratio = 1.0f;
  if (!echo_only) {
    const float* vb = vhat + (long)b * nP;
    const float* cb = cond + (long)b * nP;
    float sv = 0.f, sc = 0.f, se = 0.f;
    for (int i = threadIdx.x; i < nP; i += 256) {
      sv += vb[i] * vb[i];
      sc += cb[i] * cb[i];
    }
    for (int i = threadIdx.x; i < eP; i += 256) se += eb[i] * eb[i];
    sv = wave_sum(sv);
    sc = wave_sum(sc);
    se = wave_sum(se);
    if (lane == 0) { red[0][wv] = sv; red[1][wv] = sc; red[2][wv] = se; }
    __syncthreads();
    const float E = (red[2][0] + red[2][1]) + (red[2][2] + red[2][3]);
    const float nx = sqrtf((red[0][0] + red[0][1]) + (red[0][2] + red[0][3]) + E);
    const float nc = sqrtf((red[1][0] + red[1][1]) + (red[1][2] + red[1][3]) + E);
    ratio = fminf(fmaxf(nc / nx, renorm), 1.0f);
    __syncthreads();
  }
  auto step = [&](float xo, float v, const float* nz, long e) {
    float x0 = sp.kx * xo + sp.kv * v;
    if (sp.clip > 0.f) x0 = fminf(fmaxf(x0, -sp.clip), sp.clip);
    float xn = sp.c0 * x0 + sp.cx * xo;
    if (nz) xn += sp.sigma * nz[e];
    return xn;
  };
  if (!echo_only) {
    for (int i = threadIdx.x; i < nP; i += 256) {
      const long e = (long)b * nP + i;
      x[e] = step(x[e], ratio * vhat[e] + (extra ? extra[e] : 0.f), noise, e);
    }
  }
  for (int i = threadIdx.x; i < eP; i += 256) {
    const long e = (long)b * eP + i;
    echo[e] = step(echo[e], ratio * echo[e], echo_noise, e);
  }
}

int renorm_step(float* x, const float* vhat, const float* cond, const float* extra, const float* noise, float* echo, const float* echo_noise,
                int B, int nP, int eP, const SamplerStep& sp, float renorm, int echo_only, hipStream_t st) {
  ProfScope prof(PROF_DECODER, 0.0, st);
  if (B <= 0 || (nP <= 0 && eP <= 0)) return 0;
  if (!echo || (!echo_only && (!x || !vhat || !cond))) return set_error(NOVA_ERR_ARG, "renorm_step: null pointer");
  hipLaunchKernelGGL(renorm_step_kernel, dim3(B), dim3(256), 0, st, x, vhat, cond, extra, noise, echo, echo_noise, nP, eP, sp, renorm, echo_only);
  return check_launch("renorm_step");
}

__global__ void scale_vector_kernel(float* v, int n, float f) {
  const int i = blockIdx.x * blockDim.x + threadIdx.x;
  if (i < n) v[i] *= f;
}

int scale_vector(float* v, int n, float f, hipStream_t st) {
  ProfScope prof(PROF_DECODER, 0.0, st);
  if (n <= 0) return 0;
  hipLaunchKernelGGL(scale_vector_kernel, dim3((n + 255) / 256), dim3(256), 0, st, v, n, f);
  return check_launch("scale_vector");
}

int renorm_euler(float* x, const float* vhat, const float* cond, const float* extra, float* echo, int B, int n, int P, float dt,
                 float renorm, hipStream_t st) {
  ProfScope prof(PROF_DECODER, 0.0, st);
  if (B <= 0 || n <= 0) return 0;
  hipLaunchKernelGGL(renorm_euler_kernel, dim3(B), dim3(256), 0, st, x, vhat, cond, extra, echo, n * P, dt, renorm);
  return check_launch("renorm_euler");
}

template <typename T>
__global__ __launch_bounds__(256) void kv_append_kernel(const T* __restrict__ qkv, T* __restrict__ cache, long rows, int Lq,
                                                        int D, long cap, long base) {
  const int lane = threadIdx.x & 63;
  const long row = (long)blockIdx.x * 4 + (threadIdx.x >> 6);
  if (row >= rows) return;
  const long s = row / Lq, l = row - s * Lq;
  const T* src = qkv + row * 3 * D + D;
  T* dst = cache + (s * cap + base + l) * 2 * D;
  constexpr int V = 16 / sizeof(T);
  for (int d = lane * V; d < 2 * D; d += 64 * V) *reinterpret_cast<u4v*>(dst + d) = *reinterpret_cast<const u4v*>(src + d);
}

int kv_append(const void* qkv, void* cache, int S, int Lq, int D, long cap, long base, int dtype, hipStream_t st) {
  ProfScope prof(PROF_TOKENS, 0.0, st);
  const long rows = (long)S * Lq;
  if (rows <= 0) return 0;
  const int V = dtype_is16(dtype) ? 8 : 4;
  if (D % V) return set_error(NOVA_ERR_SHAPE, "kv_append: D must be a multiple of %d", V);
  if (base < 0 || base + Lq > cap) return set_error(NOVA_ERR_SHAPE, "kv_append: rows [%ld, %ld) exceed the cache capacity %ld", base, base + Lq, cap);
  dim3 grid((unsigned)((rows + 3) / 4)), block(256);
  dispatch_dtype(dtype, [&](auto tag) {
    using T = decltype(tag);
    hipLaunchKernelGGL(kv_append_kernel<T>, grid, block, 0, st, (const T*)qkv, (T*)cache, rows, Lq, D, cap, base);
    return 0;
  });
  return check_launch("kv_append");
}

template <typename T>
__global__ __launch_bounds__(256) void modulate_rows_kernel(const T* __restrict__ x, const T* __restrict__ mod, T* __restrict__ out,
                                                            long total4, int D) {
  for (long i = (long)blockIdx.x * blockDim.x + threadIdx.x; i < total4; i += (long)gridDim.x * blockDim.x) {
    const long e = i * 4;
    const long r = e / D;
    const int d = (int)(e - r * D);
    const f4v xv = Vec4<T>::load(x + e);
    const f4v sc = Vec4<T>::load(mod + r * 2 * D + d), sh = Vec4<T>::load(mod + r * 2 * D + D + d);
    Vec4<T>::store(out + e, xv * (1.0f + sc) + sh);
  }
}

int modulate_rows(const void* x, const void* mod, void* out, long rows, int D, int dtype, hipStream_t st) {
  ProfScope prof(PROF_TOKENS, 0.0, st);
  if (rows <= 0) return 0;
  if (D % 4) return set_error(NOVA_ERR_SHAPE, "modulate_rows: D %% 4 != 0");
  const long total4 = rows * D / 4;
  const int blocks = (int)((total4 + 255) / 256 > 8192 ? 8192 : (total4 + 255) / 256);
  dispatch_dtype(dtype, [&](auto tag) {
    using T = decltype(tag);
    hipLaunchKernelGGL(modulate_rows_kernel<T>, dim3(blocks), dim3(256), 0, st, (const T*)x, (const T*)mod, (T*)out, total4, D);
    return 0;
  });
  return check_launch("modulate_rows");
}

}
```

nova_pointcloud_amd/hip.py:

```python

import ctypes
import os
import threading

import torch

F32, BF16, F16 = 0, 1, 2
ACT_NONE, ACT_GELU_ERF, ACT_SILU = 0, 1, 2

_LIB_PATH = os.path.join(os.path.dirname(os.path.abspath(__file__)), "libnova_hip.so")
_lock = threading.Lock()
_lib = None
_device_ok = False

c_void_p, c_int, c_long, c_float = ctypes.c_void_p, ctypes.c_int, ctypes.c_long, ctypes.c_float


class NovaHipError(RuntimeError):
    """Raised when libnova_hip.so is missing, mis-built, or a call into it fails."""


class VitBlock(ctypes.Structure):

    _fields_ = [(k, c_void_p) for k in (
        "qkv_w", "qkv_b", "proj_w", "proj_b", "norm1_w", "norm1_b",
        "fc1_w", "fc1_b", "fc2_w", "fc2_b", "norm2_w", "norm2_b")]


class VitBlockFp8(ctypes.Structure):

    _fields_ = [(k, c_void_p) for k in ("qkv_w8", "qkv_ws", "fc1_w8", "fc1_ws", "fc2_w8", "fc2_ws")]


class MlpBlock(ctypes.Structure):

    _fields_ = [(k, c_void_p) for k in ("fc1_w", "fc1_b", "fc2_w", "fc2_b", "norm2_w", "norm2_b")]


class Decoder(ctypes.Structure):

    _fields_ = [("depth", c_int), ("blocks", ctypes.POINTER(MlpBlock))] + [(k, c_void_p) for k in (
        "adaln_w", "adaln_b", "patch_w", "patch_b", "head_w", "head_b")]


class SamplerStep(ctypes.Structure):

    _fields_ = [(k, c_float) for k in ("guidance", "kx", "kv", "clip", "c0", "cx", "sigma", "extra_scale")] + [("extra_kind", c_int)]


SIGNATURES = {
    "nova_gemm_bias_act": [c_void_p] * 4 + [c_int] * 5 + [c_void_p],
    "nova_qkv_rope": [c_void_p] * 5 + [c_int] * 6 + [c_void_p],
    "nova_quantize_rows_fp8": [c_void_p] * 3 + [ctypes.c_longlong, c_int, c_void_p],
    "nova_gemm_fp8_bias_act": [c_void_p] * 6 + [c_int] * 4 + [c_void_p],
    "nova_qkv_rope_cols": [c_void_p] * 5 + [c_int] * 8 + [c_void_p],
    "nova_rope_table": [c_void_p] * 3 + [c_int] * 5 + [c_void_p, c_void_p],
    "nova_attn_fwd": [c_void_p] * 4 + [c_int] * 5 + [c_long] * 3 + [c_float, c_int, c_void_p],
    "nova_row_norm": [c_void_p] * 5 + [c_long] + [c_int] * 3 + [c_void_p, c_void_p, c_long, c_int, c_float, c_int, c_void_p],
    "nova_embed_canvas": [c_void_p] * 7 + [c_int] * 5 + [c_void_p],
    "nova_build_sequence": [c_void_p, c_long, c_void_p, c_long, c_void_p, c_void_p] + [c_int] * 6 + [c_void_p],
    "nova_scatter_tokens": [c_void_p] * 3 + [c_int] * 7 + [c_void_p],
    "nova_silu_add_rows": [c_void_p] * 3 + [c_long, c_int, c_int, c_void_p],
    "nova_timestep_freq": [c_void_p] * 3 + [c_int] * 3 + [c_void_p],
    "nova_patch_embed_rows": [c_void_p] * 4 + [c_int] * 6 + [c_void_p],
    "nova_head_cfg_euler": [c_void_p] * 4 + [c_int] * 4 + [c_float, c_int, c_float, c_int, c_void_p],
    "nova_vit_blocks_forward": [ctypes.POINTER(VitBlock), c_int, c_void_p] + [c_int] * 5 + [c_void_p, c_int]
    + [c_void_p] * 4 + [c_int, c_void_p],
    "nova_row_norm_fp8": [c_void_p] * 7 + [c_long, c_int, c_float, c_void_p],
    "nova_gemm_fp8_gelu_q8": [c_void_p] * 6 + [c_int] * 3 + [c_void_p, c_void_p, c_void_p],
    "nova_qkv_rope_fp8": [c_void_p] * 7 + [c_int] * 5 + [c_float, c_void_p],
    "nova_vit_blocks_forward_fp8": [ctypes.POINTER(VitBlock), ctypes.POINTER(VitBlockFp8), c_int, c_void_p] + [c_int] * 5
    + [c_void_p, c_int] + [c_void_p] * 10 + [c_void_p],
    "nova_vit_blocks_forward_kv": [ctypes.POINTER(VitBlock), c_int, c_void_p] + [c_int] * 5 + [c_void_p, c_int]
    + [c_void_p, c_long, c_long] + [c_void_p] * 4 + [c_int, c_void_p],
    "nova_pointset_nn_dist": [c_void_p] * 3 + [c_int] * 3 + [c_float, c_float, c_int, c_void_p],
    "nova_pointset_pairwise_dist": [c_void_p] * 3 + [c_int] * 3 + [c_float, c_float, c_void_p],
    "nova_pointset_chamfer_matrix": [c_void_p] * 3 + [c_int] * 6 + [c_void_p],
    "nova_pointset_emd_matrix": [c_void_p] * 3 + [c_int] * 4 + [c_void_p],
    "nova_pointset_occupancy_grid": [c_void_p] * 5 + [c_int] * 5 + [c_void_p],
    "nova_modulate_rows": [c_void_p] * 3 + [c_long, c_int, c_int, c_void_p],
    "nova_attn_fwd_lse": [c_void_p] * 5 + [c_int, c_int, c_int, c_int, c_long, c_long, c_void_p, c_void_p],
    "nova_attn_bwd": [c_void_p] * 10 + [c_int, c_int, c_int, c_int, c_long, c_long, c_long, c_long, c_float, c_void_p, c_void_p],
    "nova_row_norm_bwd": [c_void_p] * 5 + [c_long, c_int, c_int, c_int] + [c_void_p] * 4 + [c_int, c_long, c_int, c_float, c_int, c_void_p],
    "nova_act_fwd": [c_void_p, c_void_p, ctypes.c_longlong, c_int, c_int, c_void_p],
    "nova_act_bwd": [c_void_p, c_void_p, c_void_p, ctypes.c_longlong, c_int, c_int, c_void_p],
    "nova_row_norm_chain": [c_void_p] * 5 + [c_long, c_int, c_int, c_int, c_float, c_float, c_void_p, c_void_p, c_long, c_int, c_int, c_void_p],
    "nova_adaln_fc1": [c_void_p, c_void_p, c_long, c_int, c_int, c_float, c_void_p, c_void_p, c_void_p, c_void_p, c_long]
    + [c_int] * 4 + [c_void_p],
    "nova_decoder_denoise": [ctypes.POINTER(Decoder), c_void_p, c_void_p, c_void_p, c_void_p, c_void_p, c_float, c_void_p]
    + [c_int] * 6 + [c_void_p] * 7 + [c_int, c_int, c_void_p],
    "nova_decoder_denoise_echo": [ctypes.POINTER(Decoder), c_void_p, c_void_p, c_void_p, c_void_p, c_void_p, c_float, c_void_p, c_void_p]
    + [c_int] * 7 + [c_void_p] * 7 + [c_int, c_int, c_void_p],
}
SIGNATURES["nova_prof_enable"] = [c_int]
SIGNATURES["nova_debug_force_gemm_tile"] = [c_int]
SIGNATURES["nova_debug_set_graphs"] = [c_int]
SIGNATURES["nova_debug_set_attn_variant"] = [c_int]
SIGNATURES["nova_debug_drop_graphs"] = []
SIGNATURES["nova_debug_graph_stats"] = [ctypes.POINTER(c_long), ctypes.POINTER(c_long)]
SIGNATURES["nova_prof_collect"] = [ctypes.POINTER(ctypes.c_double), ctypes.POINTER(ctypes.c_double),
                                   ctypes.POINTER(ctypes.c_longlong), c_int]
PROF_SLOTS = ["gemm_bias", "gemm_bias_gelu", "gemm_bias_silu", "qkv_gemm_rope", "attention", "row_norm", "gemm_small_tile", "gemm_bias_wide_k",
              "token_plumbing", "decoder_glue"]
PLAIN = {"nova_version": (c_int, []), "nova_last_error": (ctypes.c_char_p, []), "nova_check_device": (c_int, [])}


def lib_path() -> str:
    return _LIB_PATH


ABI_VERSION = 404


def load(check_device=True):
    global _lib, _device_ok
    with _lock:
        if _lib is None:
            if not os.path.exists(_LIB_PATH):
                raise NovaHipError(
                    f"{_LIB_PATH} not found: the HIP extension is not built. Run "
                    "`python -c 'import __graft_entry__ as g; g.build()'` (or `make -C nova_pointcloud_amd/csrc`). "
                    "There is no CPU fallback for the generation path."
                )
            try:
                lib = ctypes.CDLL(_LIB_PATH)
            except OSError as e:
                raise NovaHipError(f"cannot load {_LIB_PATH}: {e}") from e
            lib.nova_version.restype = c_int
            if lib.nova_version() != ABI_VERSION:
                raise NovaHipError(f"{_LIB_PATH} is C ABI version {lib.nova_version()}, this package binds version {ABI_VERSION} "
                                   "(include/nova_hip.h NOVA_HIP_VERSION): rebuild it with `make -C nova_pointcloud_amd/csrc`")
            for name, argtypes in SIGNATURES.items():
                fn = getattr(lib, name)
                fn.argtypes, fn.restype = argtypes, c_int
            for name, (res, argtypes) in PLAIN.items():
                fn = getattr(lib, name)
                fn.argtypes, fn.restype = argtypes, res
            _lib = lib
        if check_device and not _device_ok:
            if not torch.cuda.is_available():
                raise NovaHipError("no GPU visible: libnova_hip needs an MI355X (gfx950) device")
            rc = _lib.nova_check_device()
            if rc != 0:
                raise NovaHipError(_lib.nova_last_error().decode())
            _device_ok = True
    return _lib


def call(name, *args):
    lib = _lib if (_lib is not None and _device_ok) else load()
    rc = getattr(lib, name)(*args)
    if rc != 0:
        raise NovaHipError(f"{name} failed ({rc}): {lib.nova_last_error().decode()}")


def dtype_code(dtype: torch.dtype) -> int:
    if dtype == torch.float32:
        return F32
    if dtype == torch.bfloat16:
        return BF16
    if dtype == torch.float16:
        return F16
    raise NovaHipError(f"libnova_hip supports float32, bfloat16 and float16 activations, got {dtype}")


def stream_ptr() -> int:
    return torch.cuda.current_stream().cuda_stream


def ptr(t, dtype=None):
    if t is None:
        return None
    if not t.is_cuda:
        raise NovaHipError("libnova_hip got a CPU tensor")
    if not t.is_contiguous():
        raise NovaHipError("libnova_hip needs contiguous tensors")
    if dtype is not None and t.dtype != dtype:
        raise NovaHipError(f"expected {dtype}, got {t.dtype}")
    return t.data_ptr()


def gemm_bias_act(a, w, bias=None, act=ACT_NONE, out=None):
    M, K = a.shape
    N = w.shape[0]
    assert w.shape[1] == K and w.dtype == a.dtype
    out = a.new_empty(M, N) if out is None else out
    call("nova_gemm_bias_act", ptr(a), ptr(w), ptr(bias, torch.float32), ptr(out), M, N, K, act,
         dtype_code(a.dtype), stream_ptr())
    return out


def qkv_rope(x, w, bias, rope, S, L, heads, out=None):
    D = x.shape[-1]
    out = x.new_empty(S * L, 3 * D) if out is None else out
    nb = rope.shape[0] if rope is not None else 1
    if rope is not None:
        assert rope.shape[1] == L and rope.shape[2] * 2 == D // heads
    call("nova_qkv_rope", ptr(x), ptr(w), ptr(bias, torch.float32), ptr(rope, torch.float32), ptr(out),
         S, L, D, heads, nb, dtype_code(x.dtype), stream_ptr())
    return out


def quantize_rows_fp8(x):
    rows, D = x.shape
    q = torch.empty(rows, D, dtype=torch.uint8, device=x.device)
    scale = torch.empty(rows, dtype=torch.float32, device=x.device)
    call("nova_quantize_rows_fp8", ptr(x, torch.bfloat16), ptr(q), ptr(scale), rows, D, stream_ptr())
    return q, scale


def gemm_fp8_bias_act(a8, a_scale, w8, w_scale, bias, act=0, out=None):
    M, K = a8.shape
    N = w8.shape[0]
    out = torch.empty(M, N, dtype=torch.bfloat16, device=a8.device) if out is None else out
    call("nova_gemm_fp8_bias_act", ptr(a8), ptr(a_scale, torch.float32), ptr(w8), ptr(w_scale, torch.float32),
         ptr(bias, torch.float32), ptr(out), M, N, K, act, stream_ptr())
    return out


def rope_table(pos, ids, pad, inv_freq, nb, hd, out=None):
    n_pos = pos.shape[0]
    n_tok = ids.shape[1] if ids is not None else n_pos
    if out is None:
        out = torch.empty(nb, pad + n_tok, hd // 2, 2, dtype=torch.float32, device=pos.device)
    else:
        out = out[: nb * (pad + n_tok) * hd].view(nb, pad + n_tok, hd // 2, 2)
    call("nova_rope_table", ptr(pos, torch.float32), ptr(ids, torch.int64), ptr(out), nb, pad, n_tok, n_pos, hd,
         ptr(inv_freq, torch.float32), stream_ptr())
    return out


def attn_fwd(q, k, v, out, S, heads, Lq, Lk, hd, q_rs, kv_rs, o_rs, scale=None, k_off=0, v_off=0):
    es = q.element_size()
    assert k.dtype == q.dtype and v.dtype == q.dtype and out.dtype == q.dtype
    call("nova_attn_fwd", ptr(q), ptr(k) + k_off * es, ptr(v) + v_off * es, ptr(out), S, heads, Lq, Lk, hd, q_rs, kv_rs, o_rs,
         float(hd) ** -0.5 if scale is None else float(scale), dtype_code(q.dtype), stream_ptr())
    return out


def attn_fwd_packed(qkv, S, L, heads, out=None):
    D = qkv.shape[-1] // 3
    out = qkv.new_empty(S * L, D) if out is None else out
    return attn_fwd(qkv, qkv, qkv, out, S, heads, L, L, D // heads, 3 * D, 3 * D, D, k_off=D, v_off=2 * D)


def qkv_rope_cols(x, w, bias, rope, L, hd, rope_cols, out=None):
    M, K = x.shape
    N = w.shape[0]
    assert w.shape[1] == K and w.dtype == x.dtype
    if rope is not None:
        assert rope.shape[1] == L and rope.shape[2] * 2 == hd
    out = x.new_empty(M, N) if out is None else out
    call("nova_qkv_rope_cols", ptr(x), ptr(w), ptr(bias, torch.float32), ptr(rope, torch.float32), ptr(out), M, N, K, L,
         rope.shape[0] if rope is not None else 1, hd, rope_cols, dtype_code(x.dtype), stream_ptr())
    return out


def modulate_rows(x, mod, out=None):
    rows, D = x.shape
    assert mod.shape == (rows, 2 * D) and mod.dtype == x.dtype
    out = torch.empty_like(x) if out is None else out
    call("nova_modulate_rows", ptr(x), ptr(mod), ptr(out), rows, D, dtype_code(x.dtype), stream_ptr())
    return out


def vit_blocks_forward_kv(blocks, x, S, L, heads, hidden, rope, cache, cache_cap, cache_len, ws_qkv, ws_a, ws_b, ws_h):
    D = x.shape[-1]
    call("nova_vit_blocks_forward_kv", blocks, len(blocks), ptr(x), S, L, D, heads, hidden, ptr(rope, torch.float32),
         rope.shape[0] if rope is not None else 1, ptr(cache), cache_cap, cache_len, ptr(ws_qkv), ptr(ws_a), ptr(ws_b),
         ptr(ws_h), dtype_code(x.dtype), stream_ptr())
    return x


def row_norm(x, out=None, gamma=None, beta=None, mod=None, scale_off=-1, shift_off=-1, gate_off=-1, res=None,
             gather=None, eps=1e-5, rows=None):
    D = x.shape[-1]
    rows = (gather.numel() if gather is not None else x.numel() // D) if rows is None else rows
    out = x.new_empty(rows, D) if out is None else out
    mod_ld = mod.shape[-1] if mod is not None else 0
    call("nova_row_norm", ptr(x), ptr(out), ptr(gamma, torch.float32), ptr(beta, torch.float32), ptr(mod), mod_ld,
         scale_off, shift_off, gate_off, ptr(res), ptr(gather, torch.int32), rows, D, float(eps),
         dtype_code(x.dtype), stream_ptr())
    return out


def adaln_fc1(x, mod, scale_off, shift_off, w, bias=None, act=ACT_SILU, eps=1e-6, out=None):
    rows, D = x.shape
    N = w.shape[0]
    out = x.new_empty(rows, N) if out is None else out
    h = x.new_empty(rows, D)
    call("nova_adaln_fc1", ptr(x), ptr(mod), mod.shape[-1], scale_off, shift_off, float(eps), ptr(w), ptr(bias, torch.float32),
         ptr(h), ptr(out), rows, N, D, act, dtype_code(x.dtype), stream_ptr())
    return out


def set_graphs(on=True):
    call("nova_debug_set_graphs", 1 if on else 0)


def graph_stats():
    c, r = c_long(0), c_long(0)
    call("nova_debug_graph_stats", ctypes.byref(c), ctypes.byref(r))
    return c.value, r.value


def prof_enable(on=True):
    call("nova_prof_enable", 1 if on else 0)


def prof_collect():
    n = len(PROF_SLOTS)
    ms, work, cnt = (ctypes.c_double * n)(), (ctypes.c_double * n)(), (ctypes.c_longlong * n)()
    call("nova_prof_collect", ms, work, cnt, n)
    return {PROF_SLOTS[i]: (ms[i], work[i], cnt[i]) for i in range(n)}
```

Measured before the change: 8304 points/s.

## Fuse decoder step boundary and add wider K-stage 64-tile GEMM

At the end of each denoise step, one new kernel now does the last block's gated residual norm, the final modulate norm, the head dot products with CFG combine, the sampler update, and the next step's patch embedding plus first modulate norm. This removes several launches and intermediate round trips per step, and a debug toggle plus a graph-key field are added for it. Separately, the 64-tile GEMM gains a KW template parameter that stages two K sub-tiles per pipeline stage, now the default for that tile, and a narrow variant is picked when the grid exceeds twice the CU count. N values that are a multiple of 64 but not 128 are also allowed on the 64 tile. The fused kernel runs its head projection one wave per row and its patch embedding through scalar loops, which may be slower than the separate kernels.

```diff
diff --git a/include/nova_hip.h b/include/nova_hip.h
--- a/include/nova_hip.h
+++ b/include/nova_hip.h
@@ -5,7 +5,7 @@
 extern "C" {
 #endif
 
-#define NOVA_HIP_VERSION 404
+#define NOVA_HIP_VERSION 405
 
 typedef enum { NOVA_F32 = 0, NOVA_BF16 = 1, NOVA_F16 = 2 } nova_dtype;
 typedef enum { NOVA_ACT_NONE = 0, NOVA_ACT_GELU_ERF = 1, NOVA_ACT_SILU = 2 } nova_act;
@@ -32,6 +32,7 @@
 int nova_debug_set_graphs(int on);
 int nova_debug_graph_stats(long* captures, long* replays);
 int nova_debug_drop_graphs(void);
+int nova_debug_set_decoder_fusion(int on);
 
 int nova_gemm_bias_act(const void* A, const void* W, const float* bias, void* out, int M, int N, int K, int act,
                        int dtype, void* stream);
diff --git a/nova_pointcloud_amd/csrc/capi.hip b/nova_pointcloud_amd/csrc/capi.hip
--- a/nova_pointcloud_amd/csrc/capi.hip
+++ b/nova_pointcloud_amd/csrc/capi.hip
@@ -105,7 +105,7 @@
 
 int nova_debug_force_gemm_tile(int tile) {
   NOVA_REQUIRE(gemm_force_tile(tile) == 0, NOVA_ERR_ARG,
-               "force_gemm_tile: this build knows 0 (auto), 16 (small-M kernel; 161 / 162 / 164 with 16 / 32 / 64 rows per workgroup), 64 / 128 (the small-M tile kernels), 256 (persistent), 257 (one tile per workgroup) and 258 (persistent, prologue form); experiment codes need the NOVA_EXPERIMENTS build");
+               "force_gemm_tile: this build knows 0 (auto), 16 (small-M kernel; 161 / 162 / 164 with 16 / 32 / 64 rows per workgroup), 64 / 128 (the small-M tile kernels; 641: the 64 tile with 128-byte K-tiles), 256 (persistent), 257 (one tile per workgroup) and 258 (persistent, prologue form); experiment codes need the NOVA_EXPERIMENTS build");
   return 0;
 }
 
@@ -473,6 +473,8 @@
 
 namespace nova {
 
+static std::atomic<int> g_boundary_fused{1};
+
 static int decoder_denoise_launches(const nova_decoder* dec, const void* zc, const void* temb, float* x, const nova_sampler_step* sched,
                                     const float* noise, float renorm, float* echo_energy, int steps, int S, int B, int n, int P, int D,
                                     void* ws_a, void* ws_u, void* ws_h, void* ws_f, void* ws_g, void* ws_mod, float* ws_v, int mod_steps,
@@ -490,6 +492,9 @@
     NOVA_TRY(gemm_bias_act(ws_a, dec->adaln_w, dec->adaln_b, ws_mod, (int)(rows_all * steps), (int)mod_ld, D, NOVA_ACT_NONE, dtype, st));
   }
   void* const ws_mod_base = ws_mod;
+  const bool fuse_boundary = g_boundary_fused.load(std::memory_order_relaxed) && hoist && !do_renorm && decoder_boundary_fits(P, D, dtype);
+  auto passes_of = [&](int i) { return sched[i].guidance > 1.0f ? (sched[i].extra_kind ? 3 : 2) : 1; };
+  bool embedded = false, m1_done = false;
   for (int i = 0; i < steps; ++i) {
     const SamplerStep sp{sched[i].guidance, sched[i].kx,    sched[i].kv,          sched[i].clip,      sched[i].c0,
                          sched[i].cx,       sched[i].sigma, sched[i].extra_scale, sched[i].extra_kind};
@@ -508,13 +513,13 @@
       NOVA_TRY(silu_add_rows(zc, static_cast<const char*>(temb) + (size_t)i * D * es, ws_a, rows, D, dtype, st));
       NOVA_TRY(gemm_bias_act(ws_a, dec->adaln_w, dec->adaln_b, ws_mod, (int)rows, (int)mod_ld, D, NOVA_ACT_NONE, dtype, st));
     }
-    NOVA_TRY(patch_embed_rows(x, dec->patch_w, dec->patch_b, ws_u, Se, B, n, P, D, dtype, st));
+    if (!embedded) NOVA_TRY(patch_embed_rows(x, dec->patch_w, dec->patch_b, ws_u, Se, B, n, P, D, dtype, st));
     const bool m1_fused = gemm_modulate_fused((int)rows, D, D, dtype);
     const bool chain = !m1_fused && dtype_is16(dtype);
     for (int b = 0; b < depth; ++b) {
       const nova_mlp_block& blk = dec->blocks[b];
       RowNormArgs m1{ws_u, ws_h, nullptr, nullptr, ws_mod, mod_ld, b * 3 * D, b * 3 * D + D, -1, nullptr, nullptr, rows, D, 1e-6f};
-      if (chain && b > 0) {
+      if ((chain && b > 0) || (b == 0 && m1_done)) {
         NOVA_TRY(gemm_bias_act(ws_h, blk.fc1_w, blk.fc1_b, ws_f, (int)rows, D, D, NOVA_ACT_SILU, dtype, st));
       } else {
         NOVA_TRY(gemm_modulate_act(m1, blk.fc1_w, blk.fc1_b, ws_f, (int)rows, D, D, NOVA_ACT_SILU, dtype, st));
@@ -522,7 +527,26 @@
       NOVA_TRY(gemm_bias_act(ws_f, blk.fc2_w, blk.fc2_b, ws_g, (int)rows, D, D, NOVA_ACT_NONE, dtype, st));
       RowNormArgs m2{ws_g, ws_u, blk.norm2_w, blk.norm2_b, ws_mod, mod_ld, -1, -1, b * 3 * D + 2 * D, ws_u, nullptr, rows, D, 1e-5f};
       RowNormArgs mf{ws_u, ws_h, nullptr, nullptr, ws_mod, mod_ld, depth * 3 * D, depth * 3 * D + D, -1, nullptr, nullptr, rows, D, 1e-6f};
-      if (b == depth - 1 && dtype_is16(dtype)) {
+      if (b == depth - 1 && fuse_boundary) {
+        const float* nz = (noise && sp.sigma != 0.f) ? noise + (size_t)i * nP : nullptr;
+        DecoderBoundaryArgs ba{m2, mf, dec->head_w, dec->head_b, x, nz, sp, 0, 0, 0, dec->patch_w, dec->patch_b, ws_u, RowNormArgs{}, B, n, P, D};
+        embedded = m1_done = false;
+        if (i + 1 < steps) {
+          NOVA_REQUIRE(sched[i + 1].extra_kind >= 0 && sched[i + 1].extra_kind <= 2, NOVA_ERR_ARG, "decoder_denoise: extra_kind must be 0, 1 or 2");
+          ba.embed = 1;
+          ba.next_passes = passes_of(i + 1);
+          NOVA_REQUIRE(S >= ba.next_passes * B, NOVA_ERR_SHAPE, "decoder_denoise: step %d needs %d guidance passes but S = %d, B = %d", i + 1,
+                       ba.next_passes, S, B);
+          const long rows_next = (long)ba.next_passes * B * n;
+          ba.do_m1 = gemm_modulate_fused((int)rows_next, D, D, dtype) ? 0 : 1;
+          const void* mod_next = static_cast<char*>(ws_mod_base) + (size_t)(i + 1) * rows_all * mod_ld * es;
+          ba.m1 = RowNormArgs{ws_u, ws_h, nullptr, nullptr, mod_next, mod_ld, 0, D, -1, nullptr, nullptr, rows_next, D, 1e-6f};
+          embedded = true;
+          m1_done = ba.do_m1 != 0;
+        }
+        NOVA_TRY(decoder_boundary(ba, dtype, st));
+        continue;
+      } else if (b == depth - 1 && dtype_is16(dtype)) {
         NOVA_TRY(row_norm_chain(m2, mf, nullptr, dtype, st));
       } else if (chain) {
         RowNormArgs m1n{ws_u, ws_h, nullptr, nullptr, ws_mod, mod_ld, (b + 1) * 3 * D, (b + 1) * 3 * D + D, -1, nullptr, nullptr, rows, D, 1e-6f};
@@ -532,6 +556,7 @@
         if (b == depth - 1) NOVA_TRY(row_norm(mf, dtype, st));
       }
     }
+    if (fuse_boundary) continue;
     const void* head_in = ws_h;
     const float* nz = (noise && sp.sigma != 0.f) ? noise + (size_t)i * nP : nullptr;
     if (do_renorm && echo_rows) {
@@ -598,6 +623,11 @@
     g_graph_epoch.fetch_add(1);
     g_dec_graphs.clear();
   }
+  return 0;
+}
+
+int nova_debug_set_decoder_fusion(int on) {
+  g_boundary_fused.store(on ? 1 : 0);
   return 0;
 }
 
@@ -640,7 +670,8 @@
   for (int i = 0; i < steps; ++i) key_put(key, sched[i]);
   const void* ptrs[] = {zc, temb, x, ws_a, ws_u, ws_h, ws_f, ws_g, ws_mod, (const void*)st};
   key_put(key, ptrs);
-  const int ints[] = {steps, S, B, n, P, D, mod_steps, dtype, walk_is_reverse() ? 1 : 0, gemm_forced_tile(), skinny_forced_row_blocks()};
+  const int ints[] = {steps, S, B, n, P, D, mod_steps, dtype, walk_is_reverse() ? 1 : 0, gemm_forced_tile(), skinny_forced_row_blocks(),
+                      g_boundary_fused.load(std::memory_order_relaxed)};
   key_put(key, ints);
   auto it = g_dec_graphs.execs.find(key);
   if (it == g_dec_graphs.execs.end()) {
diff --git a/nova_pointcloud_amd/csrc/gemm.hip b/nova_pointcloud_amd/csrc/gemm.hip
--- a/nova_pointcloud_amd/csrc/gemm.hip
+++ b/nova_pointcloud_amd/csrc/gemm.hip
@@ -43,13 +43,14 @@
 #ifndef NOVA_GEMM64_STAGES
 #define NOVA_GEMM64_STAGES 2
 #endif
-template <typename T, int EPI, int F = 4>
+template <typename T, int EPI, int F = 4, int KW = 1>
 __global__ __launch_bounds__(256, 2) void gemm_kernel(const T* __restrict__ A, const T* __restrict__ W,
                                                        T* __restrict__ C, int M, int N, int K, int ntm,
                                                        int ntn, GemmEpi e) {
   constexpr int BM = 32 * F, BN = 32 * F, TILE_BYTES = BM * ROWB, WT = 16 * F;
-  constexpr int NST = F == 2 ? NOVA_GEMM64_STAGES : 2;
-  __shared__ __attribute__((aligned(16))) char smem[NST * 2 * TILE_BYTES];
+  constexpr int NST = (F == 2 && KW == 1) ? NOVA_GEMM64_STAGES : 2;
+  constexpr int STAGE_BYTES = KW * 2 * TILE_BYTES;
+  __shared__ __attribute__((aligned(16))) char smem[NST * STAGE_BYTES];
   const int tid = threadIdx.x, lane = tid & 63, wid = tid >> 6;
   const int wm = wid >> 1, wn = wid & 1;
 
@@ -75,17 +76,22 @@
     a_src[i] = reinterpret_cast<const char*>(A) + (size_t)am * rowbytes + c * 16;
     w_src[i] = reinterpret_cast<const char*>(W) + (size_t)(n0 + row) * rowbytes + c * 16;
   }
+  const int nsub = K / (ROWB / (int)sizeof(T));
+  const int nkt = (nsub + KW - 1) / KW;
   auto stage = [&](int buf, int kt) {
-    char* la = smem + buf * 2 * TILE_BYTES + wid * F * 1024;
-    char* lw = la + TILE_BYTES;
-#pragma unroll
-    for (int i = 0; i < F; ++i) {
-      __builtin_amdgcn_global_load_lds(a_src[i] + (size_t)kt * ROWB, NOVA_LDS_PTR(la + i * 1024), 16, 0, 0);
-      __builtin_amdgcn_global_load_lds(w_src[i] + (size_t)kt * ROWB, NOVA_LDS_PTR(lw + i * 1024), 16, 0, 0);
+#pragma unroll
+    for (int j = 0; j < KW; ++j) {
+      if (KW > 1 && kt * KW + j >= nsub) break;
+      char* la = smem + buf * STAGE_BYTES + j * 2 * TILE_BYTES + wid * F * 1024;
+      char* lw = la + TILE_BYTES;
+#pragma unroll
+      for (int i = 0; i < F; ++i) {
+        __builtin_amdgcn_global_load_lds(a_src[i] + (size_t)(kt * KW + j) * ROWB, NOVA_LDS_PTR(la + i * 1024), 16, 0, 0);
+        __builtin_amdgcn_global_load_lds(w_src[i] + (size_t)(kt * KW + j) * ROWB, NOVA_LDS_PTR(lw + i * 1024), 16, 0, 0);
+      }
     }
   };
 
-  const int nkt = K / (ROWB / (int)sizeof(T));
   const int fr = lane & 15, fg = lane >> 4;
 
   f4v bv[F];
@@ -117,20 +123,24 @@
     if constexpr (NST == 2) __syncthreads();
     else asm volatile("s_barrier" ::: "memory");
     if (kt + NST - 1 < nkt) stage((kt + NST - 1) % NST, kt + NST - 1);
-    const char* ta = smem + (kt % NST) * 2 * TILE_BYTES;
-    const char* tw = ta + TILE_BYTES;
-#pragma unroll
-    for (int kk = 0; kk < 2; ++kk) {
-      Frag<T> af[F], wf[F];
-#pragma unroll
-      for (int f = 0; f < F; ++f) {
-        af[f] = lds_frag<T>(ta, wm * WT + f * 16 + fr, fg + 4 * kk);
-        wf[f] = lds_frag<T>(tw, wn * WT + f * 16 + fr, fg + 4 * kk);
-      }
-#pragma unroll
-      for (int nf = 0; nf < F; ++nf)
-#pragma unroll
-        for (int mf = 0; mf < F; ++mf) acc[nf][mf] = mma(wf[nf], af[mf], acc[nf][mf]);
+#pragma unroll
+    for (int j = 0; j < KW; ++j) {
+      if (KW > 1 && kt * KW + j >= nsub) break;
+      const char* ta = smem + (kt % NST) * STAGE_BYTES + j * 2 * TILE_BYTES;
+      const char* tw = ta + TILE_BYTES;
+#pragma unroll
+      for (int kk = 0; kk < 2; ++kk) {
+        Frag<T> af[F], wf[F];
+#pragma unroll
+        for (int f = 0; f < F; ++f) {
+          af[f] = lds_frag<T>(ta, wm * WT + f * 16 + fr, fg + 4 * kk);
+          wf[f] = lds_frag<T>(tw, wn * WT + f * 16 + fr, fg + 4 * kk);
+        }
+#pragma unroll
+        for (int nf = 0; nf < F; ++nf)
+#pragma unroll
+          for (int mf = 0; mf < F; ++mf) acc[nf][mf] = mma(wf[nf], af[mf], acc[nf][mf]);
+      }
     }
   }
 
@@ -216,7 +226,7 @@
   } else {
     skinny_force_row_blocks(0);
   }
-  if (tile != 0 && tile != 16 && tile != 64 && tile != 128 && tile != 256 && tile != 257 && tile != 258) return -1;
+  if (tile != 0 && tile != 16 && tile != 64 && tile != 641 && tile != 128 && tile != 256 && tile != 257 && tile != 258) return -1;
   g_force_tile = tile;
   return 0;
 }
@@ -234,8 +244,9 @@
                        hipStream_t st) {
   const int kelems = ROWB / (int)sizeof(T);
   if (M <= 0) return 0;
-  if (N % 128 != 0 || K % kelems != 0 || K <= 0)
-    return set_error(NOVA_ERR_SHAPE, "gemm: need N %% 128 == 0 and K %% %d == 0 (got M=%d N=%d K=%d)", kelems, M, N, K);
+  const bool only64 = N % 128 == 64 && epi != EPI_ROPE && (g_force_tile == 0 || g_force_tile == 64 || g_force_tile == 641);
+  if ((N % 128 != 0 && !only64) || K % kelems != 0 || K <= 0)
+    return set_error(NOVA_ERR_SHAPE, "gemm: need N %% 128 == 0 (N %% 64 == 0 on the 64 tile) and K %% %d == 0 (got M=%d N=%d K=%d)", kelems, M, N, K);
   const bool can256 = N % 256 == 0 && (epi != EPI_ROPE || (e.rope_cols % 256 == 0 && e.q_cols % 256 == 0));
   if (g_force_tile >= 256 && !can256) return set_error(NOVA_ERR_SHAPE, "gemm: 256-tile kernel needs N %% 256 == 0");
   const long tiles256 = (long)((M + 255) / 256) * (N / 256);
@@ -249,15 +260,26 @@
   const T* w = static_cast<const T*>(W);
   T* c = static_cast<T*>(C);
   static const bool tile64_ok = [] { const char* v = getenv("NOVA_GEMM_TILE64"); return !(v && v[0] == '0'); }();
-  if (g_force_tile == 64 || (tile64_ok && g_force_tile == 0 && epi != EPI_ROPE && (long)ntm * ntn * 4 <= (long)gemm256_cu_count() * 3)) {
+  if (only64 && !tile64_ok) return set_error(NOVA_ERR_SHAPE, "gemm: N = %d needs the 64 tile", N);
+  if (only64 || g_force_tile == 64 || g_force_tile == 641 || (tile64_ok && g_force_tile == 0 && epi != EPI_ROPE && (long)ntm * ntn * 4 <= (long)gemm256_cu_count() * 3)) {
     if (epi == EPI_ROPE) return set_error(NOVA_ERR_SHAPE, "gemm: the 64 tile has no RoPE epilogue");
     ntm = (M + 63) / 64;
     ntn = N / 64;
     dim3 grid64(ntm * ntn), block(256);
+    const bool narrow = g_force_tile == 641 || (g_force_tile == 0 && (long)ntm * ntn > 2L * gemm256_cu_count());
+    if (narrow) {
+      switch (epi) {
+        case EPI_NONE: hipLaunchKernelGGL((gemm_kernel<T, EPI_NONE, 2>), grid64, block, 0, st, a, w, c, M, N, K, ntm, ntn, e); break;
+        case EPI_GELU: hipLaunchKernelGGL((gemm_kernel<T, EPI_GELU, 2>), grid64, block, 0, st, a, w, c, M, N, K, ntm, ntn, e); break;
+        case EPI_SILU: hipLaunchKernelGGL((gemm_kernel<T, EPI_SILU, 2>), grid64, block, 0, st, a, w, c, M, N, K, ntm, ntn, e); break;
+        default: return set_error(NOVA_ERR_ARG, "gemm: unknown epilogue %d", epi);
+      }
+      return check_launch("gemm (64 tile, 128-byte K-tiles)");
+    }
     switch (epi) {
-      case EPI_NONE: hipLaunchKernelGGL((gemm_kernel<T, EPI_NONE, 2>), grid64, block, 0, st, a, w, c, M, N, K, ntm, ntn, e); break;
-      case EPI_GELU: hipLaunchKernelGGL((gemm_kernel<T, EPI_GELU, 2>), grid64, block, 0, st, a, w, c, M, N, K, ntm, ntn, e); break;
-      case EPI_SILU: hipLaunchKernelGGL((gemm_kernel<T, EPI_SILU, 2>), grid64, block, 0, st, a, w, c, M, N, K, ntm, ntn, e); break;
+      case EPI_NONE: hipLaunchKernelGGL((gemm_kernel<T, EPI_NONE, 2, 2>), grid64, block, 0, st, a, w, c, M, N, K, ntm, ntn, e); break;
+      case EPI_GELU: hipLaunchKernelGGL((gemm_kernel<T, EPI_GELU, 2, 2>), grid64, block, 0, st, a, w, c, M, N, K, ntm, ntn, e); break;
+      case EPI_SILU: hipLaunchKernelGGL((gemm_kernel<T, EPI_SILU, 2, 2>), grid64, block, 0, st, a, w, c, M, N, K, ntm, ntn, e); break;
       default: return set_error(NOVA_ERR_ARG, "gemm: unknown epilogue %d", epi);
     }
     return check_launch("gemm (64 tile)");
diff --git a/nova_pointcloud_amd/csrc/nova_internal.h b/nova_pointcloud_amd/csrc/nova_internal.h
--- a/nova_pointcloud_amd/csrc/nova_internal.h
+++ b/nova_pointcloud_amd/csrc/nova_internal.h
@@ -107,6 +107,24 @@
 };
 int head_cfg_step(const void* h, const void* w, const float* bias, float* x, const float* noise, float* vhat, float* cond,
                   float* extra, int B, int n, int P, int D, const SamplerStep& sp, int defer, int dtype, hipStream_t st);
+struct DecoderBoundaryArgs {
+  RowNormArgs m2, mf;
+  const void* head_w;
+  const float* head_b;
+  float* x;
+  const float* noise;
+  SamplerStep sp;
+  int embed;
+  int next_passes;
+  int do_m1;
+  const void* patch_w;
+  const float* patch_b;
+  void* u;
+  RowNormArgs m1;
+  int B, n, P, D;
+};
+bool decoder_boundary_fits(int P, int D, int dtype);
+int decoder_boundary(const DecoderBoundaryArgs& a, int dtype, hipStream_t st);
 int scale_vector(float* v, int n, float f, hipStream_t st);
 int renorm_euler(float* x, const float* vhat, const float* cond, const float* extra, float* echo, int B, int n, int P, float dt,
                  float renorm, hipStream_t st);
diff --git a/nova_pointcloud_amd/csrc/rowops.hip b/nova_pointcloud_amd/csrc/rowops.hip
--- a/nova_pointcloud_amd/csrc/rowops.hip
+++ b/nova_pointcloud_amd/csrc/rowops.hip
@@ -458,6 +458,50 @@
 }
 
 template <typename T>
+__device__ __forceinline__ void head_dot(const T* __restrict__ w_p, const T* hc, const T* hu, const T* h3, int lane, int D, int cfg, int kind,
+                                         float& ac, float& au, float& a3) {
+  ac = 0.f, au = 0.f, a3 = 0.f;
+  for (int d = lane * 4; d < D; d += 256) {
+    const f4v wv = Vec4<T>::load(w_p + d);
+    const f4v c4 = Vec4<T>::load(hc + d);
+    ac += (wv[0] * c4[0] + wv[1] * c4[1]) + (wv[2] * c4[2] + wv[3] * c4[3]);
+    if (cfg) {
+      const f4v u4 = Vec4<T>::load(hu + d);
+      au += (wv[0] * u4[0] + wv[1] * u4[1]) + (wv[2] * u4[2] + wv[3] * u4[3]);
+    }
+    if (kind) {
+      const f4v t4 = Vec4<T>::load(h3 + d);
+      a3 += (wv[0] * t4[0] + wv[1] * t4[1]) + (wv[2] * t4[2] + wv[3] * t4[3]);
+    }
+  }
+}
+
+__device__ __forceinline__ void head_combine(float& ac, float au, float a3, float bias_p, const SamplerStep& sp, int cfg, int kind, float& vv,
+                                             float& ex) {
+  ac = wave_sum(ac) + bias_p;
+  vv = ac, ex = 0.f;
+  if (cfg) {
+    au = wave_sum(au) + bias_p;
+    if (kind) a3 = wave_sum(a3) + bias_p;
+    if (kind == 1) {
+      vv = au + (ac - a3) * sp.guidance;
+      ex = (a3 - au) * sp.extra_scale;
+    } else {
+      vv = au + (ac - au) * sp.guidance;
+      if (kind == 2) ex = (ac - a3) * sp.extra_scale;
+    }
+  }
+}
+
+__device__ __forceinline__ float sampler_step(const SamplerStep& sp, float xo, float vv, const float* __restrict__ noise, long e) {
+  float x0 = sp.kx * xo + sp.kv * vv;
+  if (sp.clip > 0.f) x0 = fminf(fmaxf(x0, -sp.clip), sp.clip);
+  float xn = sp.c0 * x0 + sp.cx * xo;
+  if (noise) xn += sp.sigma * noise[e];
+  return xn;
+}
+
+template <typename T>
 __global__ __launch_bounds__(256) void head_cfg_step_kernel(const T* __restrict__ h, const T* __restrict__ w,
                                                             const float* __restrict__ bias, float* __restrict__ x,
                                                             const float* __restrict__ noise, float* __restrict__ vhat,
@@ -472,33 +516,9 @@
   const T* hu = h + ((long)B * n + row) * D;
   const T* h3 = h + ((long)2 * B * n + row) * D;
   for (int p = 0; p < P; ++p) {
-    float ac = 0.f, au = 0.f, a3 = 0.f;
-    for (int d = lane * 4; d < D; d += 256) {
-      const f4v wv = Vec4<T>::load(w + (long)p * D + d);
-      const f4v c4 = Vec4<T>::load(hc + d);
-      ac += (wv[0] * c4[0] + wv[1] * c4[1]) + (wv[2] * c4[2] + wv[3] * c4[3]);
-      if (cfg) {
-        const f4v u4 = Vec4<T>::load(hu + d);
-        au += (wv[0] * u4[0] + wv[1] * u4[1]) + (wv[2] * u4[2] + wv[3] * u4[3]);
-      }
-      if (kind) {
-        const f4v t4 = Vec4<T>::load(h3 + d);
-        a3 += (wv[0] * t4[0] + wv[1] * t4[1]) + (wv[2] * t4[2] + wv[3] * t4[3]);
-      }
-    }
-    ac = wave_sum(ac) + bias[p];
-    float vv = ac, ex = 0.f;
-    if (cfg) {
-      au = wave_sum(au) + bias[p];
-      if (kind) a3 = wave_sum(a3) + bias[p];
-      if (kind == 1) {
-        vv = au + (ac - a3) * sp.guidance;
-        ex = (a3 - au) * sp.extra_scale;
-      } else {
-        vv = au + (ac - au) * sp.guidance;
-        if (kind == 2) ex = (ac - a3) * sp.extra_scale;
-      }
-    }
+    float ac, au, a3, vv, ex;
+    head_dot<T>(w + (long)p * D, hc, hu, h3, lane, D, cfg, kind, ac, au, a3);
+    head_combine(ac, au, a3, bias[p], sp, cfg, kind, vv, ex);
     if (lane == 0) {
       const long e = row * P + p;
       if (defer) {
@@ -506,13 +526,7 @@
         cond[e] = ac;
         if (extra) extra[e] = ex;
       } else {
-        vv += ex;
-        const float xo = x[e];
-        float x0 = sp.kx * xo + sp.kv * vv;
-        if (sp.clip > 0.f) x0 = fminf(fmaxf(x0, -sp.clip), sp.clip);
-        float xn = sp.c0 * x0 + sp.cx * xo;
-        if (noise) xn += sp.sigma * noise[e];
-        x[e] = xn;
+        x[e] = sampler_step(sp, x[e], vv + ex, noise, e);
       }
     }
   }
@@ -535,6 +549,115 @@
   });
   return check_launch("head_cfg_step");
 }
+
+template <typename T, int NIT>
+__global__ __launch_bounds__(256) void decoder_boundary_kernel(DecoderBoundaryArgs a) {
+  using C = Chunk<T>;
+  __shared__ __attribute__((aligned(16))) T hs[4][3][NIT * 512];
+  __shared__ float xs[4][64];
+  const int lane = threadIdx.x & 63, wid = threadIdx.x >> 6;
+  const long rows = (long)a.B * a.n;
+  long row = (long)blockIdx.x * 4 + wid;
+  const bool live = row < rows;
+  if (!live) row = rows - 1;
+  const int D = a.D, P = a.P;
+  const int cfg = a.sp.guidance > 1.0f;
+  const int kind = cfg ? a.sp.extra_kind : 0;
+  const int passes = cfg ? (kind ? 3 : 2) : 1;
+  for (int q = 0; q < passes; ++q) {
+    RowChainRegs<T, NIT> g;
+    row_chain_load<T, NIT>(a.m2, a.mf, q * rows + row, lane, g);
+    u4v xn[NIT];
+    C y[NIT];
+    row_chain_finish<T, NIT>(a.m2, a.mf, lane, g, xn, y);
+#pragma unroll
+    for (int it = 0; it < NIT; ++it) {
+      const int d = (it * 64 + lane) * 8;
+      if (d < D) y[it].store(&hs[wid][q][d]);
+    }
+  }
+  __syncthreads();
+  for (int p = 0; p < P; ++p) {
+    float ac, au, a3, vv, ex;
+    head_dot<T>(static_cast<const T*>(a.head_w) + (long)p * D, hs[wid][0], hs[wid][1], hs[wid][2], lane, D, cfg, kind, ac, au, a3);
+    head_combine(ac, au, a3, a.head_b[p], a.sp, cfg, kind, vv, ex);
+    const long e = row * P + p;
+    const float xnew = sampler_step(a.sp, a.x[e], vv + ex, a.noise, e);
+    if (lane == 0) {
+      xs[wid][p] = xnew;
+      if (live) a.x[e] = xnew;
+    }
+  }
+  if (!a.embed) return;
+  __syncthreads();
+  const T* pw = static_cast<const T*>(a.patch_w);
+  RowRegs<T, NIT, false, true> g1;
+#pragma unroll
+  for (int it = 0; it < NIT; ++it) {
+    const int d = (it * 64 + lane) * 8;
+    if (d < D) {
+      float e8[8];
+#pragma unroll
+      for (int k = 0; k < 8; ++k) {
+        float e = a.patch_b[d + k];
+        for (int p = 0; p < P; ++p) e += xs[wid][p] * to_f<T>(pw[(long)(d + k) * P + p]);
+        e8[k] = e;
+      }
+      g1.x[it] = u4v{Half16<T>::pack(e8[0], e8[1]), Half16<T>::pack(e8[2], e8[3]), Half16<T>::pack(e8[4], e8[5]), Half16<T>::pack(e8[6], e8[7])};
+    }
+  }
+  for (int q = 0; q < a.next_passes; ++q) {
+    const long r = q * rows + row;
+    if (live) {
+#pragma unroll
+      for (int it = 0; it < NIT; ++it) {
+        const int d = (it * 64 + lane) * 8;
+        if (d < D) *reinterpret_cast<u4v*>(static_cast<T*>(a.u) + r * D + d) = g1.x[it];
+      }
+    }
+    if (a.do_m1) {
+      row_norm_load<T, NIT, false, true>(a.m1, r, lane, g1, false);
+      C y[NIT];
+      row_norm_finish<T, NIT, false, true>(a.m1, lane, g1, y);
+      if (live) {
+#pragma unroll
+        for (int it = 0; it < NIT; ++it) {
+          const int d = (it * 64 + lane) * 8;
+          if (d < D) y[it].store(static_cast<T*>(a.m1.out) + r * D + d);
+        }
+      }
+    }
+  }
+}
+
+int decoder_boundary(const DecoderBoundaryArgs& a, int dtype, hipStream_t st) {
+  ProfScope prof(PROF_DECODER, 0.0, st);
+  const long rows = (long)a.B * a.n;
+  if (rows <= 0) return 0;
+  if (!decoder_boundary_fits(a.P, a.D, dtype)) return set_error(NOVA_ERR_SHAPE, "decoder_boundary: 16-bit rows, D %% 8 == 0, D <= 2048, P <= 64");
+  if (a.sp.extra_kind < 0 || a.sp.extra_kind > 2) return set_error(NOVA_ERR_ARG, "decoder_boundary: extra_kind must be 0, 1 or 2");
+  if (!a.m2.in || !a.m2.res || !a.m2.mod || a.m2.gate_off < 0 || a.m2.scale_off >= 0 || a.m2.gather || !a.mf.mod || a.mf.scale_off < 0 ||
+      a.mf.shift_off < 0 || a.mf.gate_off >= 0 || a.mf.gamma || a.mf.res || a.mf.gather || (a.m2.gamma == nullptr) != (a.m2.beta == nullptr) ||
+      a.m2.D != a.D || a.mf.D != a.D || !a.head_w || !a.head_b || !a.x)
+    return set_error(NOVA_ERR_ARG, "decoder_boundary: first norm = gate + residual, second = scale / shift modulate, then the head");
+  if (a.embed && (!a.patch_w || !a.patch_b || !a.u || a.next_passes < 1 || a.next_passes > 3 ||
+                  (a.do_m1 && (!a.m1.mod || !a.m1.out || a.m1.scale_off < 0 || a.m1.shift_off < 0 || a.m1.gate_off >= 0 || a.m1.gamma || a.m1.res ||
+                               a.m1.gather || a.m1.D != a.D))))
+    return set_error(NOVA_ERR_ARG, "decoder_boundary: the next step needs the patch embedding, 1 .. 3 passes and a scale / shift modulate");
+  if (a.m2.mod_ld % 8 || a.m2.gate_off % 8 || a.mf.mod_ld % 8 || a.mf.scale_off % 8 || a.mf.shift_off % 8 ||
+      (a.embed && a.do_m1 && (a.m1.mod_ld % 8 || a.m1.scale_off % 8 || a.m1.shift_off % 8)))
+    return set_error(NOVA_ERR_SHAPE, "decoder_boundary: modulation offsets must be multiples of 8");
+  const dim3 grid((unsigned)((rows + 3) / 4));
+  dispatch_half(dtype, [&](auto tag) {
+    using T = decltype(tag);
+    if ((a.D / 8 + 63) / 64 <= 2) hipLaunchKernelGGL((decoder_boundary_kernel<T, 2>), grid, dim3(256), 0, st, a);
+    else hipLaunchKernelGGL((decoder_boundary_kernel<T, 4>), grid, dim3(256), 0, st, a);
+    return 0;
+  });
+  return check_launch("decoder_boundary");
+}
+
+bool decoder_boundary_fits(int P, int D, int dtype) { return dtype_is16(dtype) && D % 8 == 0 && D <= 2048 && P > 0 && P <= 64; }
 
 __global__ __launch_bounds__(256) void renorm_euler_kernel(float* __restrict__ x, const float* __restrict__ vhat,
                                                           const float* __restrict__ cond, const float* __restrict__ extra,
diff --git a/nova_pointcloud_amd/hip.py b/nova_pointcloud_amd/hip.py
--- a/nova_pointcloud_amd/hip.py
+++ b/nova_pointcloud_amd/hip.py
@@ -97,6 +97,7 @@
 SIGNATURES["nova_debug_set_graphs"] = [c_int]
 SIGNATURES["nova_debug_set_attn_variant"] = [c_int]
 SIGNATURES["nova_debug_drop_graphs"] = []
+SIGNATURES["nova_debug_set_decoder_fusion"] = [c_int]
 SIGNATURES["nova_debug_graph_stats"] = [ctypes.POINTER(c_long), ctypes.POINTER(c_long)]
 SIGNATURES["nova_prof_collect"] = [ctypes.POINTER(ctypes.c_double), ctypes.POINTER(ctypes.c_double),
                                    ctypes.POINTER(ctypes.c_longlong), c_int]
@@ -109,7 +110,7 @@
     return _LIB_PATH
 
 
-ABI_VERSION = 404
+ABI_VERSION = 405
 
 
 def load(check_device=True):
```

Measured after the change: 8334 points/s, median of 6. No clear change (+0.4%).
